# lukifer23/Matrix0

Measured on NVIDIA B200. Metric: MCTS sims/sec, batched self-play, ResNet-24 (BASELINE configs[3]), higher is better.
Workload: dtype fp16

## Files before the change

### matrix0_b200/csrc/nn_fused_kernels.cu

```cuda
#include "nn.cuh"
#include <cuda_fp16.h>

namespace m0 {

__device__ __forceinline__ float fk_act(float x, int act) {
  switch (act) {
    case ACT_RELU: return x > 0.0f ? x : 0.0f;
    case ACT_SILU: return __fdividef(x, 1.0f + __expf(-x));
    default: return x;
  }
}
__device__ __forceinline__ __nv_bfloat16 fk_half(float x, int fp16) {
  if (fp16) {
    __half h = __float2half_rn(x);
    return *reinterpret_cast<__nv_bfloat16*>(&h);
  }
  return __float2bfloat16(x);
}

__device__ __forceinline__ void unpack_half8(const uint4& u, int fp16, float (&f)[8]) {
  const uint32_t w[4] = {u.x, u.y, u.z, u.w};
#pragma unroll
  for (int i = 0; i < 4; ++i) {
    if (fp16) {
      const float2 t = __half22float2(*reinterpret_cast<const __half2*>(&w[i]));
      f[2 * i] = t.x; f[2 * i + 1] = t.y;
    } else {
      const float2 t = __bfloat1622float2(*reinterpret_cast<const __nv_bfloat162*>(&w[i]));
      f[2 * i] = t.x; f[2 * i + 1] = t.y;
    }
  }
}
__device__ __forceinline__ uint32_t fk_pack2(float a, float b, int fp16) {
  if (fp16) {
    __half2 h = __floats2half2_rn(a, b);
    return *reinterpret_cast<uint32_t*>(&h);
  }
  __nv_bfloat162 t = __floats2bfloat162_rn(a, b);
  return *reinterpret_cast<uint32_t*>(&t);
}

__global__ void __launch_bounds__(320, 2)
se_apply_gn_kernel(const __nv_bfloat16* __restrict__ conv_out, const float* __restrict__ gate, float* __restrict__ x,
                   const float* __restrict__ gamma, const float* __restrict__ beta, __nv_bfloat16* __restrict__ a_out, int C, int act, int fp16) {
  __shared__ float s_part[8][40][2];
  const int b = blockIdx.x;
  const int nq = C >> 3;
  const int q = threadIdx.x % nq, rg = threadIdx.x / nq;
  const size_t base = (size_t)b * 64 * C + (size_t)rg * 8 * C + 8 * q;
  float v[8][8];
  if (conv_out) {
    float e[8];
    if (gate) {
      const float4 e0 = *reinterpret_cast<const float4*>(gate + (size_t)b * C + 8 * q);
      const float4 e1 = *reinterpret_cast<const float4*>(gate + (size_t)b * C + 8 * q + 4);
      e[0] = e0.x; e[1] = e0.y; e[2] = e0.z; e[3] = e0.w; e[4] = e1.x; e[5] = e1.y; e[6] = e1.z; e[7] = e1.w;
    } else {
#pragma unroll
      for (int j = 0; j < 8; ++j) e[j] = 1.0f;
    }
    uint4 cv[8];
#pragma unroll
    for (int r = 0; r < 8; ++r) cv[r] = __ldg(reinterpret_cast<const uint4*>(conv_out + base + (size_t)r * C));
#pragma unroll
    for (int r = 0; r < 8; ++r) {
      const float4 x0 = *reinterpret_cast<const float4*>(x + base + (size_t)r * C);
      const float4 x1 = *reinterpret_cast<const float4*>(x + base + (size_t)r * C + 4);
      float c[8];
      unpack_half8(cv[r], fp16, c);
      v[r][0] = fmaf(c[0], e[0], x0.x); v[r][1] = fmaf(c[1], e[1], x0.y); v[r][2] = fmaf(c[2], e[2], x0.z); v[r][3] = fmaf(c[3], e[3], x0.w);
      v[r][4] = fmaf(c[4], e[4], x1.x); v[r][5] = fmaf(c[5], e[5], x1.y); v[r][6] = fmaf(c[6], e[6], x1.z); v[r][7] = fmaf(c[7], e[7], x1.w);
    }
#pragma unroll
    for (int r = 0; r < 8; ++r) {
      *reinterpret_cast<float4*>(x + base + (size_t)r * C) = make_float4(v[r][0], v[r][1], v[r][2], v[r][3]);
      *reinterpret_cast<float4*>(x + base + (size_t)r * C + 4) = make_float4(v[r][4], v[r][5], v[r][6], v[r][7]);
    }
  } else {
#pragma unroll
    for (int r = 0; r < 8; ++r) {
      const float4 x0 = *reinterpret_cast<const float4*>(x + base + (size_t)r * C);
      const float4 x1 = *reinterpret_cast<const float4*>(x + base + (size_t)r * C + 4);
      v[r][0] = x0.x; v[r][1] = x0.y; v[r][2] = x0.z; v[r][3] = x0.w; v[r][4] = x1.x; v[r][5] = x1.y; v[r][6] = x1.z; v[r][7] = x1.w;
    }
  }
  if (!a_out) return;
  __nv_bfloat16* ao = a_out + base;
  if (!gamma) {
#pragma unroll
    for (int r = 0; r < 8; ++r)
      *reinterpret_cast<uint4*>(ao + (size_t)r * C) = make_uint4(fk_pack2(v[r][0], v[r][1], fp16), fk_pack2(v[r][2], v[r][3], fp16),
                                                                 fk_pack2(v[r][4], v[r][5], fp16), fk_pack2(v[r][6], v[r][7], fp16));
    return;
  }
  float s = 0.f;
#pragma unroll
  for (int r = 0; r < 8; ++r) s += ((v[r][0] + v[r][1]) + (v[r][2] + v[r][3])) + ((v[r][4] + v[r][5]) + (v[r][6] + v[r][7]));
  s += __shfl_xor_sync(0xFFFFFFFFu, s, 1);
  s_part[rg][q][0] = s;
  __syncthreads();
  float tot = 0.f;
#pragma unroll
  for (int g = 0; g < 8; ++g) tot += s_part[g][q][0];
  const float mean = tot * (1.0f / 1024.0f);
  float d2 = 0.f;
#pragma unroll
  for (int r = 0; r < 8; ++r)
#pragma unroll
    for (int j = 0; j < 8; ++j) {
      const float a = v[r][j] - mean;
      d2 = fmaf(a, a, d2);
    }
  d2 += __shfl_xor_sync(0xFFFFFFFFu, d2, 1);
  s_part[rg][q][1] = d2;
  __syncthreads();
  float vs = 0.f;
#pragma unroll
  for (int g = 0; g < 8; ++g) vs += s_part[g][q][1];
  const float rstd = rsqrtf(vs * (1.0f / 1024.0f) + 1e-5f);
  float gsc[8], bsh[8];
  {
    const float4 g0 = *reinterpret_cast<const float4*>(gamma + 8 * q), g1 = *reinterpret_cast<const float4*>(gamma + 8 * q + 4);
    const float4 b0 = *reinterpret_cast<const float4*>(beta + 8 * q), b1 = *reinterpret_cast<const float4*>(beta + 8 * q + 4);
    const float gg[8] = {g0.x, g0.y, g0.z, g0.w, g1.x, g1.y, g1.z, g1.w};
    const float bb[8] = {b0.x, b0.y, b0.z, b0.w, b1.x, b1.y, b1.z, b1.w};
#pragma unroll
    for (int j = 0; j < 8; ++j) { gsc[j] = gg[j] * rstd; bsh[j] = bb[j] - mean * gsc[j]; }
  }
#pragma unroll
  for (int r = 0; r < 8; ++r) {
    float y[8];
#pragma unroll
    for (int j = 0; j < 8; ++j) y[j] = fk_act(fmaf(v[r][j], gsc[j], bsh[j]), act);
    *reinterpret_cast<uint4*>(ao + (size_t)r * C) =
        make_uint4(fk_pack2(y[0], y[1], fp16), fk_pack2(y[2], y[3], fp16), fk_pack2(y[4], y[5], fp16), fk_pack2(y[6], y[7], fp16));
  }
}

__global__ void __launch_bounds__(320, 2)
gn_act_res_kernel(const float* __restrict__ x, const float* __restrict__ gamma, const float* __restrict__ beta, const float* __restrict__ residual,
                  long long residual_bstride, float* __restrict__ out, __nv_bfloat16* __restrict__ out_half, int C, int act, int fp16) {
  __shared__ float s_part[8][40][2];
  const int b = blockIdx.x;
  const int nq = C >> 3;
  const int q = threadIdx.x % nq, rg = threadIdx.x / nq;
  const size_t off = (size_t)rg * 8 * C + 8 * q;
  const size_t base = (size_t)b * 64 * C + off;
  float v[8][8];
#pragma unroll
  for (int r = 0; r < 8; ++r) {
    const float4 x0 = *reinterpret_cast<const float4*>(x + base + (size_t)r * C);
    const float4 x1 = *reinterpret_cast<const float4*>(x + base + (size_t)r * C + 4);
    v[r][0] = x0.x; v[r][1] = x0.y; v[r][2] = x0.z; v[r][3] = x0.w; v[r][4] = x1.x; v[r][5] = x1.y; v[r][6] = x1.z; v[r][7] = x1.w;
  }
  float s = 0.f;
#pragma unroll
  for (int r = 0; r < 8; ++r) s += ((v[r][0] + v[r][1]) + (v[r][2] + v[r][3])) + ((v[r][4] + v[r][5]) + (v[r][6] + v[r][7]));
  s += __shfl_xor_sync(0xFFFFFFFFu, s, 1);
  s_part[rg][q][0] = s;
  __syncthreads();
  float tot = 0.f;
#pragma unroll
  for (int g = 0; g < 8; ++g) tot += s_part[g][q][0];
  const float mean = tot * (1.0f / 1024.0f);
  float d2 = 0.f;
#pragma unroll
  for (int r = 0; r < 8; ++r)
#pragma unroll
    for (int j = 0; j < 8; ++j) {
      const float a = v[r][j] - mean;
      d2 = fmaf(a, a, d2);
    }
  d2 += __shfl_xor_sync(0xFFFFFFFFu, d2, 1);
  s_part[rg][q][1] = d2;
  __syncthreads();
  float vs = 0.f;
#pragma unroll
  for (int g = 0; g < 8; ++g) vs += s_part[g][q][1];
  const float rstd = rsqrtf(vs * (1.0f / 1024.0f) + 1e-5f);
  float gsc[8], bsh[8];
  {
    const float4 g0 = *reinterpret_cast<const float4*>(gamma + 8 * q), g1 = *reinterpret_cast<const float4*>(gamma + 8 * q + 4);
    const float4 b0 = *reinterpret_cast<const float4*>(beta + 8 * q), b1 = *reinterpret_cast<const float4*>(beta + 8 * q + 4);
    const float gg[8] = {g0.x, g0.y, g0.z, g0.w, g1.x, g1.y, g1.z, g1.w};
    const float bb[8] = {b0.x, b0.y, b0.z, b0.w, b1.x, b1.y, b1.z, b1.w};
#pragma unroll
    for (int j = 0; j < 8; ++j) { gsc[j] = gg[j] * rstd; bsh[j] = bb[j] - mean * gsc[j]; }
  }
  const float* rb = residual ? residual + (size_t)b * residual_bstride + off : nullptr;
#pragma unroll
  for (int r = 0; r < 8; ++r) {
    float y[8];
#pragma unroll
    for (int j = 0; j < 8; ++j) y[j] = fk_act(fmaf(v[r][j], gsc[j], bsh[j]), act);
    if (rb) {
      const float4 r0 = *reinterpret_cast<const float4*>(rb + (size_t)r * C), r1 = *reinterpret_cast<const float4*>(rb + (size_t)r * C + 4);
      y[0] += r0.x; y[1] += r0.y; y[2] += r0.z; y[3] += r0.w; y[4] += r1.x; y[5] += r1.y; y[6] += r1.z; y[7] += r1.w;
    }
    if (out) {
      *reinterpret_cast<float4*>(out + base + (size_t)r * C) = make_float4(y[0], y[1], y[2], y[3]);
      *reinterpret_cast<float4*>(out + base + (size_t)r * C + 4) = make_float4(y[4], y[5], y[6], y[7]);
    }
    if (out_half)
      *reinterpret_cast<uint4*>(out_half + base + (size_t)r * C) =
          make_uint4(fk_pack2(y[0], y[1], fp16), fk_pack2(y[2], y[3], fp16), fk_pack2(y[4], y[5], fp16), fk_pack2(y[6], y[7], fp16));
  }
}

__global__ void planes_to_nhwc_half_kernel(const float* __restrict__ planes, __nv_bfloat16* __restrict__ out, int B, int P, int fp16) {
  const size_t i = (size_t)blockIdx.x * blockDim.x + threadIdx.x;
  if (i >= (size_t)B * 64 * 64) return;
  const int c = (int)(i & 63);
  const int sq = (int)((i >> 6) & 63);
  const size_t b = i >> 12;
  out[i] = c < P ? fk_half(planes[(b * P + c) * 64 + sq], fp16) : fk_half(0.0f, fp16);
}

__global__ void __launch_bounds__(320)
se_gate_kernel(const float* __restrict__ pool, const float* __restrict__ w1t, const float* __restrict__ b1, const float* __restrict__ w2t,
               const float* __restrict__ b2, float* __restrict__ gate, int B, int C, int hid, int act) {
  extern __shared__ float sm[];
  float* s_pool = sm;
  float* s_hid = sm + 16 * C;
  float* s_red = s_hid + 16 * hid;
  const int b0 = blockIdx.x * 16, t = threadIdx.x;
  const int nb = min(16, B - b0);
  for (int i = t; i < 16 * C; i += blockDim.x) {
    const int j = i / C, c = i - j * C;
    float v = 0.f;
    if (j < nb) {
      const float* pp = pool + (size_t)(b0 + j) * 2 * C;
      v = (pp[c] + pp[C + c]) * (1.0f / 64.0f);
    }
    s_pool[c * 16 + j] = v;
  }
  __syncthreads();
  {
    const int parts = blockDim.x / hid;
    const int part = t / hid, u = t - part * hid;
    if (part < parts) {
      float h[16];
#pragma unroll
      for (int j = 0; j < 16; ++j) h[j] = 0.f;
      const int c0 = part * (C / parts), c1 = (part + 1 == parts) ? C : c0 + C / parts;
#pragma unroll 16
      for (int c = c0; c < c1; ++c) {
        const float w = __ldg(w1t + c * hid + u);
        const float4* sp = reinterpret_cast<const float4*>(s_pool + c * 16);
        const float4 p0 = sp[0], p1 = sp[1], p2 = sp[2], p3 = sp[3];
        h[0] = fmaf(w, p0.x, h[0]); h[1] = fmaf(w, p0.y, h[1]); h[2] = fmaf(w, p0.z, h[2]); h[3] = fmaf(w, p0.w, h[3]);
        h[4] = fmaf(w, p1.x, h[4]); h[5] = fmaf(w, p1.y, h[5]); h[6] = fmaf(w, p1.z, h[6]); h[7] = fmaf(w, p1.w, h[7]);
        h[8] = fmaf(w, p2.x, h[8]); h[9] = fmaf(w, p2.y, h[9]); h[10] = fmaf(w, p2.z, h[10]); h[11] = fmaf(w, p2.w, h[11]);
        h[12] = fmaf(w, p3.x, h[12]); h[13] = fmaf(w, p3.y, h[13]); h[14] = fmaf(w, p3.z, h[14]); h[15] = fmaf(w, p3.w, h[15]);
      }
      float4* dst = reinterpret_cast<float4*>(s_red + (part * hid + u) * 16);
      dst[0] = make_float4(h[0], h[1], h[2], h[3]); dst[1] = make_float4(h[4], h[5], h[6], h[7]);
      dst[2] = make_float4(h[8], h[9], h[10], h[11]); dst[3] = make_float4(h[12], h[13], h[14], h[15]);
    }
    __syncthreads();
    for (int o = t; o < hid * 16; o += blockDim.x) {
      const int u2 = o >> 4;
      float a = b1[u2];
      for (int pp = 0; pp < parts; ++pp) a += s_red[pp * hid * 16 + o];
      s_hid[o] = fk_act(a, act);
    }
    __syncthreads();
  }
  for (int c = t; c < C; c += blockDim.x) {
    float z[16];
    const float bias = b2[c];
#pragma unroll
    for (int j = 0; j < 16; ++j) z[j] = bias;
#pragma unroll 16
    for (int u = 0; u < hid; ++u) {
      const float w = __ldg(w2t + u * C + c);
      const float4* sh = reinterpret_cast<const float4*>(s_hid + u * 16);
      const float4 p0 = sh[0], p1 = sh[1], p2 = sh[2], p3 = sh[3];
      z[0] = fmaf(w, p0.x, z[0]); z[1] = fmaf(w, p0.y, z[1]); z[2] = fmaf(w, p0.z, z[2]); z[3] = fmaf(w, p0.w, z[3]);
      z[4] = fmaf(w, p1.x, z[4]); z[5] = fmaf(w, p1.y, z[5]); z[6] = fmaf(w, p1.z, z[6]); z[7] = fmaf(w, p1.w, z[7]);
      z[8] = fmaf(w, p2.x, z[8]); z[9] = fmaf(w, p2.y, z[9]); z[10] = fmaf(w, p2.z, z[10]); z[11] = fmaf(w, p2.w, z[11]);
      z[12] = fmaf(w, p3.x, z[12]); z[13] = fmaf(w, p3.y, z[13]); z[14] = fmaf(w, p3.z, z[14]); z[15] = fmaf(w, p3.w, z[15]);
    }
#pragma unroll
    for (int j = 0; j < 16; ++j)
      if (j < nb) gate[(size_t)(b0 + j) * C + c] = __fdividef(1.0f, 1.0f + __expf(-z[j]));
  }
}

int nn_se_gate(const float* pool, const float* w1t, const float* b1, const float* w2t, const float* b2, float* gate, int B, int C, int hid, int act,
               cudaStream_t s) {
  if (hid <= 0 || hid > 320) { m0_set_error("se_gate: unsupported hidden width %d", hid); return M0_ERR_ARG; }
  const int parts = 320 / hid;
  se_gate_kernel<<<(B + 15) / 16, 320, (size_t)16 * (C + hid + (size_t)parts * hid) * sizeof(float), s>>>(pool, w1t, b1, w2t, b2, gate, B, C, hid, act);
  return m0_check_launch("se_gate");
}

int nn_se_apply_gn(const __nv_bfloat16* conv_out, const float* gate, float* x, const float* gamma, const float* beta, __nv_bfloat16* a_out, int B,
                   int C, int act, cudaStream_t s) {
  if (C > 320 || C % 32 != 0) { m0_set_error("se_apply_gn: unsupported channel count %d", C); return M0_ERR_ARG; }
  if (C % 16 != 0) { m0_set_error("se_apply_gn: channels must be a multiple of 16"); return M0_ERR_ARG; }
  se_apply_gn_kernel<<<B, C, 0, s>>>(conv_out, gate, x, gamma, beta, a_out, C, act, nn_half_format());
  return m0_check_launch("se_apply_gn");
}
int nn_gn_act_res(const float* x, const float* gamma, const float* beta, const float* residual, long long residual_bstride, float* out,
                  __nv_bfloat16* out_half, int B, int C, int act, cudaStream_t s) {
  if (C > 320 || C % 16 != 0) { m0_set_error("gn_act_res: unsupported channel count %d", C); return M0_ERR_ARG; }
  if (act != ACT_NONE && act != ACT_RELU && act != ACT_SILU) { m0_set_error("gn_act_res: unsupported activation %d", act); return M0_ERR_ARG; }
  gn_act_res_kernel<<<B, C, 0, s>>>(x, gamma, beta, residual, residual_bstride, out, out_half, C, act, nn_half_format());
  return m0_check_launch("gn_act_res");
}
__global__ void se_hidden_kernel(const float* __restrict__ part, int splits, long long split_stride, const float* __restrict__ b1,
                                 __nv_bfloat16* __restrict__ hidden, int B, int hid, int ld, int act, int fp16) {
  const int i = blockIdx.x * blockDim.x + threadIdx.x;
  if (i >= B * hid) return;
  const int b = i / hid, u = i - b * hid;
  float a = b1[u];
  for (int ks = 0; ks < splits; ++ks) a += part[(size_t)ks * split_stride + (size_t)b * ld + u];
  hidden[(size_t)b * ld + u] = fk_half(fk_act(a, act), fp16);
}
int nn_se_hidden(const float* part, int splits, long long split_stride, const float* b1, __nv_bfloat16* hidden, int B, int hid, int ld, int act,
                 cudaStream_t s) {
  se_hidden_kernel<<<(B * hid + 255) / 256, 256, 0, s>>>(part, splits, split_stride, b1, hidden, B, hid, ld, act, nn_half_format());
  return m0_check_launch("se_hidden");
}
static constexpr int SE_TAIL_BOARDS = 8;
__global__ void __launch_bounds__(320, 4)
se_tail_kernel(const float* __restrict__ part, int splits, long long split_stride, int ld, const float* __restrict__ b1,
                               const float* __restrict__ w2t, const float* __restrict__ b2, float* __restrict__ gate, int B, int C, int hid, int act) {
  extern __shared__ __align__(16) float s_hid[];
  const int b0 = blockIdx.x * SE_TAIL_BOARDS;
  const int nb = min(SE_TAIL_BOARDS, B - b0);
  for (int i = threadIdx.x; i < SE_TAIL_BOARDS * hid; i += blockDim.x) {
    const int b = i / hid, u = i - b * hid;
    float a = 0.f;
    if (b < nb) {
      a = b1[u];
      for (int ks = 0; ks < splits; ++ks) a += part[(size_t)ks * split_stride + (size_t)(b0 + b) * ld + u];
      a = fk_act(a, act);
    }
    s_hid[u * SE_TAIL_BOARDS + b] = a;
  }
  __syncthreads();
  for (int c = threadIdx.x; c < C; c += blockDim.x) {
    float acc[SE_TAIL_BOARDS];
#pragma unroll
    for (int b = 0; b < SE_TAIL_BOARDS; ++b) acc[b] = 0.f;
    for (int u0 = 0; u0 < hid; u0 += 16) {
      float w[16];
#pragma unroll
      for (int k = 0; k < 16; ++k) w[k] = (u0 + k < hid) ? __ldg(w2t + (size_t)(u0 + k) * C + c) : 0.f;
#pragma unroll
      for (int k = 0; k < 16; ++k) {
        if (u0 + k >= hid) break;
        const float4 h0 = *reinterpret_cast<const float4*>(s_hid + (u0 + k) * SE_TAIL_BOARDS);
        const float4 h1 = *reinterpret_cast<const float4*>(s_hid + (u0 + k) * SE_TAIL_BOARDS + 4);
        acc[0] = fmaf(w[k], h0.x, acc[0]); acc[1] = fmaf(w[k], h0.y, acc[1]); acc[2] = fmaf(w[k], h0.z, acc[2]); acc[3] = fmaf(w[k], h0.w, acc[3]);
        acc[4] = fmaf(w[k], h1.x, acc[4]); acc[5] = fmaf(w[k], h1.y, acc[5]); acc[6] = fmaf(w[k], h1.z, acc[6]); acc[7] = fmaf(w[k], h1.w, acc[7]);
      }
    }
    const float bias = b2[c];
#pragma unroll
    for (int b = 0; b < SE_TAIL_BOARDS; ++b)
      if (b < nb) gate[(size_t)(b0 + b) * C + c] = __fdividef(1.0f, 1.0f + __expf(-(acc[b] + bias)));
  }
}
int nn_se_tail(const float* part, int splits, long long split_stride, int ld, const float* b1, const float* w2t, const float* b2, float* gate, int B,
               int C, int hid, int act, cudaStream_t s) {
  const int threads = C >= 320 ? 320 : ((C + 31) / 32 * 32);
  se_tail_kernel<<<(B + SE_TAIL_BOARDS - 1) / SE_TAIL_BOARDS, threads, (size_t)SE_TAIL_BOARDS * hid * sizeof(float), s>>>(
      part, splits, split_stride, ld, b1, w2t, b2, gate, B, C, hid, act);
  return m0_check_launch("se_tail");
}
__global__ void value_tail_kernel(const float* __restrict__ gate, const float* __restrict__ h, const float* __restrict__ w3, const float* __restrict__ b3,
                                  float* __restrict__ values, int B, int C) {
  const int b = blockIdx.x * (blockDim.x >> 5) + (threadIdx.x >> 5), lane = threadIdx.x & 31;
  if (b >= B) return;
  float acc = 0.f;
  for (int c = lane; c < C; c += 32) acc = fmaf(w3[c], h[(size_t)b * C + c] * gate[(size_t)b * C + c], acc);
  for (int off = 16; off > 0; off >>= 1) acc += __shfl_xor_sync(0xFFFFFFFFu, acc, off);
  if (lane == 0) values[b] = tanhf(acc + b3[0]);
}
int nn_value_tail(const float* gate, const float* h, const float* w3, const float* b3, float* values, int B, int C, cudaStream_t s) {
  value_tail_kernel<<<(B + 7) / 8, 256, 0, s>>>(gate, h, w3, b3, values, B, C);
  return m0_check_launch("value_tail");
}
int nn_planes_to_nhwc_half(const float* planes, __nv_bfloat16* out, int B, int P, cudaStream_t s) {
  const size_t total = (size_t)B * 64 * 64;
  planes_to_nhwc_half_kernel<<<(unsigned)((total + 255) / 256), 256, 0, s>>>(planes, out, B, P, nn_half_format());
  return m0_check_launch("planes_to_nhwc_half");
}

}
```

### matrix0_b200/csrc/nn_tc_kernels.cu

```cuda
#include "net_host.cuh"
#include "tc_gemm.cuh"
#include "tc_conv_pair.cuh"
#include <new>
#include <stdlib.h>
#include <string.h>
#include <stdio.h>
#include <string>
#include <utility>
#include <vector>

using namespace m0;

namespace m0 {
int nn_se_apply_gn(const __nv_bfloat16* conv_out, const float* gate, float* x, const float* gamma, const float* beta, __nv_bfloat16* a_out, int B,
                   int C, int act, cudaStream_t s);
int nn_planes_to_nhwc_half(const float* planes, __nv_bfloat16* out, int B, int P, cudaStream_t s);
int nn_se_hidden(const float* part, int splits, long long split_stride, const float* b1, __nv_bfloat16* hidden, int B, int hid, int ld, int act,
                 cudaStream_t s);
int nn_gn_act_res(const float* x, const float* gamma, const float* beta, const float* residual, long long residual_bstride, float* out,
                  __nv_bfloat16* out_half, int B, int C, int act, cudaStream_t s);
int nn_attention_tc(const void* qkv_half, const float* rel_bias, void* out_half, int B, int C, int heads, float mix, cudaStream_t s);
int nn_se_tail(const float* part, int splits, long long split_stride, int ld, const float* b1, const float* w2t, const float* b2, float* gate, int B,
               int C, int hid, int act, cudaStream_t s);
int nn_value_tail(const float* gate, const float* h, const float* w3, const float* b3, float* values, int B, int C, cudaStream_t s);
int nn_se_gate(const float* pool, const float* w1t, const float* b1, const float* w2t, const float* b2, float* gate, int B, int C, int hid, int act,
               cudaStream_t s);
}

namespace m0 {
__global__ void transpose_f32_kernel(const float* __restrict__ in, float* __restrict__ out, int rows, int cols) {
  int i = blockIdx.x * blockDim.x + threadIdx.x;
  if (i >= rows * cols) return;
  int r = i / cols, c = i % cols;
  out[c * rows + r] = in[i];
}
__global__ void se_fold_kernel(const float* __restrict__ conv_w, const float* __restrict__ w1, float* __restrict__ out, int C, int hid) {
  const int K = 12 * C;
  const int i = blockIdx.x * blockDim.x + threadIdx.x;
  if (i >= hid * K) return;
  const int u = i / K, k = i - u * K;
  const int ci = k % C, j = (k / C) % 6, hb = k / (6 * C);
  unsigned plus = 0, minus = 0;
  switch (j) {
    case 0: plus = 0x1FF; break;
    case 1: minus = hb ? 0x007 : 0x1C0; break;
    case 2: minus = 0x124; break;
    case 3: minus = 0x049; break;
    case 4: plus = hb ? (1u << 2) : (1u << 8); break;
    default: plus = hb ? (1u << 0) : (1u << 6); break;
  }
  float acc = 0.f;
  for (int c = 0; c < C; ++c) {
    const float* wr = conv_w + (size_t)c * 9 * C + ci;
    float wsum = 0.f;
#pragma unroll
    for (int t = 0; t < 9; ++t) {
      if (plus & (1u << t)) wsum += wr[t * C];
      if (minus & (1u << t)) wsum -= wr[t * C];
    }
    acc = fmaf(w1[u * C + c], wsum, acc);
  }
  out[i] = acc * (1.0f / 64.0f);
}
template <typename T>
__global__ void pad_cols_kernel(const T* __restrict__ in, T* __restrict__ out, int rows, int cols, int cols_pad) {
  const int i = blockIdx.x * blockDim.x + threadIdx.x;
  if (i >= rows * cols_pad) return;
  const int r = i / cols_pad, c = i - r * cols_pad;
  out[i] = c < cols ? in[r * cols + c] : T(0);
}
}

namespace {

typedef CUresult (*EncodeTiledFn)(CUtensorMap*, CUtensorMapDataType, cuuint32_t, void*, const cuuint64_t*, const cuuint64_t*, const cuuint32_t*,
                                  const cuuint32_t*, CUtensorMapInterleave, CUtensorMapSwizzle, CUtensorMapL2promotion, CUtensorMapFloatOOBfill);

EncodeTiledFn get_encode() {
  static EncodeTiledFn fn = nullptr;
  if (!fn) {
    void* p = nullptr;
    cudaDriverEntryPointQueryResult q;
    if (cudaGetDriverEntryPoint("cuTensorMapEncodeTiled", &p, cudaEnableDefault, &q) == cudaSuccess && q == cudaDriverEntryPointSuccess)
      fn = reinterpret_cast<EncodeTiledFn>(p);
  }
  return fn;
}

int make_map_2d(CUtensorMap* m, const void* ptr, uint64_t rows, uint64_t cols, uint32_t box_rows) {
  EncodeTiledFn enc = get_encode();
  if (!enc) { m0_set_error("cuTensorMapEncodeTiled is not available from the driver"); return M0_ERR_CUDA; }
  cuuint64_t dims[2] = {cols, rows};
  cuuint64_t strides[1] = {cols * 2};
  cuuint32_t box[2] = {64, box_rows};
  cuuint32_t estr[2] = {1, 1};
  CUresult r = enc(m, CU_TENSOR_MAP_DATA_TYPE_BFLOAT16, 2, const_cast<void*>(ptr), dims, strides, box, estr, CU_TENSOR_MAP_INTERLEAVE_NONE,
                   CU_TENSOR_MAP_SWIZZLE_128B, CU_TENSOR_MAP_L2_PROMOTION_L2_256B, CU_TENSOR_MAP_FLOAT_OOB_FILL_NONE);
  if (r != CUDA_SUCCESS) { m0_set_error("cuTensorMapEncodeTiled(2d %llu x %llu) failed: %d", (unsigned long long)rows, (unsigned long long)cols, (int)r); return M0_ERR_CUDA; }
  return M0_OK;
}

int make_map_nhwc(CUtensorMap* m, const void* ptr, uint64_t boards, uint64_t C, uint32_t box_x = 8) {
  EncodeTiledFn enc = get_encode();
  if (!enc) { m0_set_error("cuTensorMapEncodeTiled is not available from the driver"); return M0_ERR_CUDA; }
  cuuint64_t dims[4] = {C, 8, 8, boards};
  cuuint64_t strides[3] = {C * 2, C * 2 * 8, C * 2 * 64};
  cuuint32_t box[4] = {64, box_x, 8, 2};
  cuuint32_t estr[4] = {1, 1, 1, 1};
  CUresult r = enc(m, CU_TENSOR_MAP_DATA_TYPE_BFLOAT16, 4, const_cast<void*>(ptr), dims, strides, box, estr, CU_TENSOR_MAP_INTERLEAVE_NONE,
                   CU_TENSOR_MAP_SWIZZLE_128B, CU_TENSOR_MAP_L2_PROMOTION_L2_256B, CU_TENSOR_MAP_FLOAT_OOB_FILL_NONE);
  if (r != CUDA_SUCCESS) { m0_set_error("cuTensorMapEncodeTiled(nhwc boards=%llu C=%llu) failed: %d", (unsigned long long)boards, (unsigned long long)C, (int)r); return M0_ERR_CUDA; }
  return M0_OK;
}

int make_map_out(CUtensorMap* m, const void* ptr, uint64_t rows, uint64_t cols, bool fp32, bool swizzle64 = false) {
  EncodeTiledFn enc = get_encode();
  if (!enc) { m0_set_error("cuTensorMapEncodeTiled is not available from the driver"); return M0_ERR_CUDA; }
  cuuint64_t dims[2] = {cols, rows};
  cuuint64_t strides[1] = {cols * (fp32 ? 4 : 2)};
  cuuint32_t box[2] = {16, 32};
  cuuint32_t estr[2] = {1, 1};
  CUresult r = enc(m, fp32 ? CU_TENSOR_MAP_DATA_TYPE_FLOAT32 : CU_TENSOR_MAP_DATA_TYPE_BFLOAT16, 2, const_cast<void*>(ptr), dims, strides, box, estr,
                   CU_TENSOR_MAP_INTERLEAVE_NONE, swizzle64 ? CU_TENSOR_MAP_SWIZZLE_64B : CU_TENSOR_MAP_SWIZZLE_NONE, CU_TENSOR_MAP_L2_PROMOTION_NONE,
                   CU_TENSOR_MAP_FLOAT_OOB_FILL_NONE);
  if (r != CUDA_SUCCESS) { m0_set_error("cuTensorMapEncodeTiled(out %llu x %llu) failed: %d", (unsigned long long)rows, (unsigned long long)cols, (int)r); return M0_ERR_CUDA; }
  return M0_OK;
}

struct TcWeight {
  __nv_bfloat16* w = nullptr;
  CUtensorMap map;
  CUtensorMap map_pair;
  bool pair = false;
  int n = 0, k = 0, n_part = 0, cluster = 1;
  int n_launch = 0;
};

int pick_cluster(int n_part) {
  static int forced = -1;
  if (forced < 0) {
    const char* e = getenv("M0_TC_CLUSTER");
    forced = e ? atoi(e) : 0;
  }
  int cs = forced > 0 ? forced : 2;
  while (cs > 1 && ((n_part / cs) % 8 != 0 || n_part % cs != 0)) cs >>= 1;
  return cs;
}

struct TcBlock {
  TcWeight conv1, conv2, qkv, proj;
  TcWeight se_fold, se_w2;
};

struct TcState {
  int sm_count = 148;
  int max_smem = 0;
  size_t smem_pair[9] = {0, 0, 0, 0, 0, 0, 0, 0, 0};
  size_t smem_gemm = 0;
  TcWeight pst, inter;
  std::vector<TcBlock> blocks;
  float *pool = nullptr, *se_hid = nullptr, *se_gate = nullptr;
  std::vector<float*> se_w1t, se_w2t;
  bool se_fused = false;
  int hid_pad = 0;
  __nv_bfloat16 *prims = nullptr, *se_hid_h = nullptr;
  float* se_part = nullptr;
  int se_splits = 1;
  size_t se_rows = 0;
  CUtensorMap prims_mat, se_hid_mat;
  __nv_bfloat16* planes_h = nullptr;
  __nv_bfloat16* qkv_h = nullptr;
  bool heads_tc = false;
  TcWeight pol_conv, pol_fc1, pol_fc2, val_conv1, val_conv2, val_fc1, val_fc2, val_gate;
  bool val_tail_tc = false;
  int pol_rank_pad = 0;
  __nv_bfloat16 *ph_h = nullptr, *pf_h = nullptr, *vh_h = nullptr;
  __nv_bfloat16 *vf1_h = nullptr, *vf2_h = nullptr;
  CUtensorMap ph_mat, pf_mat, vh_conv_mat, vh_fc_mat, vf1_mat, vf2_mat;
  CUtensorMap planes_conv;
  TcWeight stem;
  int cap = 0;
  __nv_bfloat16 *a1 = nullptr, *a2 = nullptr;
  CUtensorMap a1_conv, a2_conv, a1_mat, a2_mat;
  CUtensorMap a1_convp, a2_convp, planes_convp;
  CUtensorMap x_io;
  const void* x_ptr = nullptr;
  CUtensorMap qkv_out, t2f_out;
  CUtensorMap a1_out, a2_out, t1_out, t2h_out;
  const void *t1_ptr = nullptr, *t2_ptr = nullptr;
  int out_rows = 0;
  std::vector<void*> allocs;
};

struct TcProfiler {
  struct Rec { const char* name; cudaEvent_t a, b; };
  std::vector<Rec> pending;
  std::vector<std::pair<std::string, std::pair<double, long>>> acc;
  int on = -1;
  bool enabled() {
    if (on < 0) {
      const char* e = getenv("M0_TC_PROFILE");
      on = (e && atoi(e)) ? 1 : 0;
      if (on) atexit(&TcProfiler::dump_static);
    }
    return on >= 1;
  }
  void set(int enable) { enabled(); on = enable ? 2 : 0; }
  void reset() { collect(); acc.clear(); }
  static TcProfiler& get() { static TcProfiler p; return p; }
  void begin(const char* name, cudaStream_t s) {
    Rec r; r.name = name;
    cudaEventCreate(&r.a); cudaEventCreate(&r.b);
    cudaEventRecord(r.a, s);
    pending.push_back(r);
  }
  void end(cudaStream_t s) { cudaEventRecord(pending.back().b, s); }
  void collect() {
    for (Rec& r : pending) {
      cudaEventSynchronize(r.b);
      float ms = 0.f;
      cudaEventElapsedTime(&ms, r.a, r.b);
      bool found = false;
      for (auto& kv : acc) if (kv.first == r.name) { kv.second.first += ms; kv.second.second++; found = true; break; }
      if (!found) acc.push_back({r.name, {ms, 1}});
      cudaEventDestroy(r.a); cudaEventDestroy(r.b);
    }
    pending.clear();
  }
  static void dump_static() {
    TcProfiler& p = get();
    double tot = 0;
    for (auto& kv : p.acc) tot += kv.second.first;
    fprintf(stderr, "[m0 tc profile] total %.3f ms\n", tot);
    for (auto& kv : p.acc)
      fprintf(stderr, "[m0 tc profile] %5.1f%%  n=%5ld  avg=%9.1f us  %s\n", 100.0 * kv.second.first / tot, kv.second.second,
              1e3 * kv.second.first / kv.second.second, kv.first.c_str());
  }
};
#define PROF(name, call)                                   \
  do {                                                     \
    TcProfiler& _p = TcProfiler::get();                    \
    if (_p.enabled()) {                                    \
      _p.begin(name, s);                                   \
      int _r = (call);                                     \
      _p.end(s);                                           \
      if (_r != M0_OK) return _r;                          \
    } else {                                               \
      int _r = (call);                                     \
      if (_r != M0_OK) return _r;                          \
    }                                                      \
  } while (0)

#define TRY(x)            \
  do {                    \
    int _r = (x);         \
    if (_r != M0_OK) return _r; \
  } while (0)

int n_part_for(int n) { return n <= 256 ? n : n / 2; }

int kblocks_for(int cin) { return (cin + 63) / 64; }

int env_int(const char* name, int dflt) {
  const char* e = getenv(name);
  return e ? atoi(e) : dflt;
}
int slice_width_for(int n, int dflt) {
  static int forced = -1;
  if (forced < 0) forced = env_int("M0_TC_SLICE", 0);
  if (forced > 0) return (n % forced == 0) ? forced : dflt;
  if (!env_int("M0_TC_ACC2", 1)) return dflt;
  for (int w = 256; w >= 64; w -= 16)
    if (n % w == 0) return w;
  return dflt;
}
bool pair_ok(int n) {
  static int on = -1;
  if (on < 0) on = env_int("M0_TC_PAIR", 1);
  return on && n % 32 == 0 && n >= 64 && n <= 512;
}

struct ConvFusion {
  float* resid_x = nullptr;
  const float* gate = nullptr;
  __nv_bfloat16* prims = nullptr;
  const CUtensorMap* x_map = nullptr;
};

int launch_conv_pair(TcState* st, const CUtensorMap& a_map, const TcWeight& w, int boards, int cin, float* out_f32, __nv_bfloat16* out_half,
                     int ldc, int act, cudaStream_t s, const float* gn_gamma = nullptr, const float* gn_beta = nullptr, float* pool_part = nullptr,
                     const ConvFusion* fuse = nullptr, int conv = 1, int n_slices = 1, const CUtensorMap* out_map = nullptr) {
  tc::ConvPairParams p;
  memset(&p, 0, sizeof(p));
  p.boards = boards;
  p.N = w.n_launch;
  p.kb_per_tap = kblocks_for(cin);
  p.conv = conv;
  p.n_slices = n_slices;
  if (n_slices > 1 && (gn_gamma || pool_part || fuse)) { m0_set_error("pair kernel: fused epilogues need a single slice"); return M0_ERR_ARG; }
  p.fp16 = nn_half_format();
  p.out_f32 = out_f32;
  p.out_half = out_half;
  p.ldc = ldc;
  p.act = act;
  p.gn_gamma = gn_gamma;
  p.gn_beta = gn_beta;
  p.pool_part = pool_part;
  if (fuse) { p.resid_x = fuse->resid_x; p.gate = fuse->gate; p.prims = fuse->prims; }
  static int cap = -1;
  if (cap < 0) cap = env_int("M0_TC_STAGES", 0);
  const int stage_bytes = conv ? tc::CP_A_SLOT + 3 * (w.n_launch / 4) * 128 : (w.n_launch / 4) * 128;
  const int a_res = conv ? 0 : 2 * kblocks_for(cin) * tc::A_TILE_BYTES;
  const int fz = !fuse ? 0 : fuse->resid_x ? 2 : fuse->prims ? 1 : 0;
  const int epi_bytes = fz == 2 ? tc::CP_EPI_BYTES_FUSE : tc::CP_EPI_BYTES;
  int stages = (st->max_smem - 2048 - epi_bytes - a_res) / stage_bytes;
  if (stages > 8) stages = 8;
  if (cap > 0 && stages > cap) stages = cap;
  if (stages < 2) { m0_set_error("pair convolution: stage does not fit in shared memory (N=%d)", w.n_launch); return M0_ERR_ARG; }
  p.stages = stages;
  const size_t smem = (size_t)stages * stage_bytes + a_res + epi_bytes + 1024 + 512;
  const int nch = (w.n_launch / 32 + tc::CP_CSETS - 1) / tc::CP_CSETS;
  if (nch > 4) { m0_set_error("pair kernel: N = %d is too wide", w.n_launch); return M0_ERR_ARG; }
  auto kernel = fz == 2 ? (nch <= 1 ? tc::conv_pair_kernel<1, 2> : nch <= 3 ? tc::conv_pair_kernel<3, 2> : tc::conv_pair_kernel<4, 2>)
                : fz == 1 ? (nch <= 1 ? tc::conv_pair_kernel<1, 1> : nch <= 3 ? tc::conv_pair_kernel<3, 1> : tc::conv_pair_kernel<4, 1>)
                          : (nch <= 1 ? tc::conv_pair_kernel<1, 0> : nch <= 3 ? tc::conv_pair_kernel<3, 0> : tc::conv_pair_kernel<4, 0>);
  const int kidx = (nch <= 1 ? 0 : nch <= 3 ? 1 : 2) + 3 * fz;
  if (smem > st->smem_pair[kidx]) {
    M0_CUDA_TRY(cudaFuncSetAttribute(kernel, cudaFuncAttributeMaxDynamicSharedMemorySize, (int)smem));
    st->smem_pair[kidx] = smem;
  }
  const int tiles = (boards + 3) / 4;
  int clusters = st->sm_count / 2;
  if (clusters > tiles) clusters = tiles;
  cudaLaunchConfig_t cfg;
  memset(&cfg, 0, sizeof(cfg));
  cfg.gridDim = dim3((unsigned)(clusters * 2));
  cfg.blockDim = dim3(tc::CP_THREADS);
  cfg.dynamicSmemBytes = smem;
  cfg.stream = s;
  cudaLaunchAttribute attr[1];
  attr[0].id = cudaLaunchAttributeClusterDimension;
  attr[0].val.clusterDim.x = 2;
  attr[0].val.clusterDim.y = 1;
  attr[0].val.clusterDim.z = 1;
  cfg.attrs = attr;
  cfg.numAttrs = 1;
  if (fuse && fuse->resid_x && (!fuse->x_map || (out_half && !out_map))) { m0_set_error("pair kernel: the residual epilogue needs the x and output tensor maps"); return M0_ERR_ARG; }
  p.out_tma = (out_map && !(fuse && fuse->prims)) ? 1 : 0;
  M0_CUDA_TRY(cudaLaunchKernelEx(&cfg, kernel, a_map, w.map_pair, out_map ? *out_map : a_map, (fuse && fuse->x_map) ? *fuse->x_map : a_map, p));
  return m0_check_launch("conv_pair_kernel");
}

int make_weight(TcState* st, TcWeight* out, const float* w_f32, int n, int k, int n_launch, cudaStream_t s, int taps = 1) {
  const int cin = k / taps, cin_pad = taps > 1 ? kblocks_for(cin) * 64 : cin;
  k = taps * cin_pad;
  out->n = n;
  out->k = k;
  out->n_part = n_part_for(n_launch);
  out->cluster = pick_cluster(out->n_part);
  void* p = nullptr;
  M0_CUDA_TRY(cudaMalloc(&p, (size_t)n * k * 2));
  st->allocs.push_back(p);
  out->w = (__nv_bfloat16*)p;
  if (cin_pad != cin) {
    float* padded = nullptr;
    M0_CUDA_TRY(cudaMallocAsync((void**)&padded, (size_t)n * k * 4, s));
    pad_cols_kernel<float><<<(n * k + 255) / 256, 256, 0, s>>>(w_f32, padded, n * taps, cin, cin_pad);
    int rc = m0_check_launch("pad_taps");
    if (rc == M0_OK) rc = nn_f32_to_bf16(padded, out->w, (size_t)n * k, s);
    cudaFreeAsync(padded, s);
    TRY(rc);
  } else {
    TRY(nn_f32_to_bf16(w_f32, out->w, (size_t)n * k, s));
  }
  out->n_launch = n_launch;
  out->pair = pair_ok(n_launch) && n % n_launch == 0;
  if (out->pair) TRY(make_map_2d(&out->map_pair, out->w, (uint64_t)n, (uint64_t)k, (uint32_t)(n_launch / 4)));
  return make_map_2d(&out->map, out->w, (uint64_t)n, (uint64_t)k, (uint32_t)(out->n_part / out->cluster));
}

int pow2_cols(int n) {
  int c = 32;
  while (c < n) c <<= 1;
  return c;
}

int launch_gemm(TcState* st, const CUtensorMap& a_map, const TcWeight& w, int M, int conv, int taps, int cin, int w_row0, int N, float* out_f32,
                __nv_bfloat16* out_bf16, int ldc, int col0, const float* bias, int act, float scale, cudaStream_t s,
                const float* gn_gamma = nullptr, const float* gn_beta = nullptr, float* pool_part = nullptr, int n_store = -1, int n_slices = 1,
                int k_splits = 1, long long split_stride = 0) {
  tc::GemmParams p;
  memset(&p, 0, sizeof(p));
  p.M = M;
  p.N = N;
  p.n_slices = n_slices;
  p.k_splits = k_splits;
  p.split_stride = split_stride;
  if (k_splits > 1 && (out_bf16 || bias || act != ACT_NONE || gn_gamma || pool_part || (taps * kblocks_for(cin)) % k_splits != 0 || !out_f32)) {
    m0_set_error("tensor-core GEMM: split-K needs a plain fp32 output and a K range divisible into whole k-blocks");
    return M0_ERR_ARG;
  }
  p.n_store = n_store >= 0 ? n_store : N * n_slices;
  if (w.n_part > N || N % w.n_part != 0) { m0_set_error("tensor-core GEMM: launch width %d does not match the weight map box %d", N, w.n_part); return M0_ERR_ARG; }
  p.n_part = w.n_part;
  p.taps = taps;
  p.kb_per_tap = kblocks_for(cin);
  p.conv = conv;
  p.w_row0 = w_row0;
  {
    static int acc2 = -1;
    if (acc2 < 0) acc2 = env_int("M0_TC_ACC2", 1);
    const int stride = (N + 31) / 32 * 32;
    p.acc_stages = (acc2 && 2 * stride <= 512 && !gn_gamma) ? 2 : 1;
    p.acc_stride = stride;
    p.tmem_cols = pow2_cols(p.acc_stages * stride);
  }
  p.out_f32 = out_f32;
  p.out_bf16 = out_bf16;
  p.ldc = ldc;
  p.col0 = col0;
  p.bias = bias;
  p.act = act;
  p.scale = scale;
  p.gn_gamma = gn_gamma;
  p.gn_beta = gn_beta;
  p.pool_part = pool_part;
  if ((gn_gamma || pool_part) && (w_row0 != 0 || N % 32 != 0)) { m0_set_error("fused epilogue needs the full channel range"); return M0_ERR_ARG; }
  p.cluster = w.cluster;
  p.fp16 = nn_half_format();
  const int stage_bytes = tc::A_TILE_BYTES + N * tc::BK * 2;
  int stages = (st->max_smem - 2048 - tc::EPI_STAGE_BYTES) / stage_bytes;
  if (stages > 6) stages = 6;
  {
    static int cap = -1;
    if (cap < 0) { const char* e = getenv("M0_TC_STAGES"); cap = e ? atoi(e) : 0; }
    if (cap > 0 && stages > cap) stages = cap;
  }
  if (stages < 2) { m0_set_error("tensor-core GEMM: tile does not fit in shared memory (N=%d)", N); return M0_ERR_ARG; }
  p.stages = stages;
  const size_t smem = (size_t)stages * stage_bytes + tc::EPI_STAGE_BYTES + 1024 + 256;
  if (smem > st->smem_gemm) {
    M0_CUDA_TRY(cudaFuncSetAttribute(tc::gemm_tc_kernel, cudaFuncAttributeMaxDynamicSharedMemorySize, (int)smem));
    st->smem_gemm = smem;
  }
  const int tiles = (M + tc::BM - 1) / tc::BM;
  const int cs = w.cluster;
  const int groups = (tiles + cs - 1) / cs;
  int clusters = st->sm_count / cs;
  if (clusters > groups * n_slices * k_splits) clusters = groups * n_slices * k_splits;
  cudaLaunchConfig_t cfg;
  memset(&cfg, 0, sizeof(cfg));
  cfg.gridDim = dim3((unsigned)(clusters * cs));
  cfg.blockDim = dim3(tc::NUM_THREADS);
  cfg.dynamicSmemBytes = smem;
  cfg.stream = s;
  cudaLaunchAttribute attr[1];
  attr[0].id = cudaLaunchAttributeClusterDimension;
  attr[0].val.clusterDim.x = (unsigned)cs;
  attr[0].val.clusterDim.y = 1;
  attr[0].val.clusterDim.z = 1;
  cfg.attrs = attr;
  cfg.numAttrs = 1;
  M0_CUDA_TRY(cudaLaunchKernelEx(&cfg, tc::gemm_tc_kernel, a_map, w.map, p));
  return m0_check_launch("gemm_tc_kernel");
}

int conv3x3(TcState* st, const CUtensorMap& a_map, const CUtensorMap& a_map_pair, const TcWeight& w, int B, int cin, float* out_f32,
            __nv_bfloat16* out_half, int act, cudaStream_t s, const float* gn_gamma = nullptr, const float* gn_beta = nullptr,
            float* pool_part = nullptr, const ConvFusion* fuse = nullptr, const CUtensorMap* out_map = nullptr) {
  if (w.pair) return launch_conv_pair(st, a_map_pair, w, B, cin, out_f32, out_half, w.n, act, s, gn_gamma, gn_beta, pool_part, fuse, 1, 1, out_map);
  if (fuse) { m0_set_error("fused SE / residual epilogue needs the CTA-pair convolution"); return M0_ERR_ARG; }
  return launch_gemm(st, a_map, w, B * 64, 1, 9, cin, 0, w.n, out_f32, out_half, w.n, 0, nullptr, act, 1.0f, s, gn_gamma, gn_beta, pool_part);
}

int gemm_rows64(TcState* st, const CUtensorMap& a_mat, const TcWeight& w, int B, int cin, float* out_f32, __nv_bfloat16* out_half, int ldc,
                cudaStream_t s, const CUtensorMap* out_map = nullptr) {
  const int n_slices = w.n / w.n_launch;
  static int pg = -1;
  if (pg < 0) pg = env_int("M0_TC_PAIR_GEMM", 0);
  if (pg && w.pair && cin <= 320)
    return launch_conv_pair(st, a_mat, w, B, cin, out_f32, out_half, ldc, ACT_NONE, s, nullptr, nullptr, nullptr, nullptr, 0, n_slices, out_map);
  return launch_gemm(st, a_mat, w, B * 64, 0, 1, cin, 0, w.n_launch, out_f32, out_half, ldc, 0, nullptr, ACT_NONE, 1.0f, s, nullptr, nullptr, nullptr, -1,
                     n_slices);
}

int tc_reserve(m0_net* n, TcState* st, int B) {
  const int need = (B + 1) & ~1;
  if (need <= st->cap) return M0_OK;
  const size_t C = n->cfg.channels;
  if (st->a1) cudaFree(st->a1);
  if (st->a2) cudaFree(st->a2);
  if (st->pool) cudaFree(st->pool);
  if (st->se_hid) cudaFree(st->se_hid);
  if (st->se_gate) cudaFree(st->se_gate);
  if (st->planes_h) cudaFree(st->planes_h);
  if (st->qkv_h) cudaFree(st->qkv_h);
  if (st->ph_h) cudaFree(st->ph_h);
  if (st->pf_h) cudaFree(st->pf_h);
  if (st->vh_h) cudaFree(st->vh_h);
  if (st->vf1_h) cudaFree(st->vf1_h);
  if (st->vf2_h) cudaFree(st->vf2_h);
  st->vf1_h = st->vf2_h = nullptr;
  if (st->prims) cudaFree(st->prims);
  if (st->se_hid_h) cudaFree(st->se_hid_h);
  if (st->se_part) cudaFree(st->se_part);
  st->se_part = nullptr;
  st->prims = st->se_hid_h = nullptr;
  st->qkv_h = st->ph_h = st->pf_h = st->vh_h = nullptr;
  st->a1 = st->a2 = nullptr;
  st->pool = st->se_hid = st->se_gate = nullptr;
  st->planes_h = nullptr;
  st->cap = 0;
  M0_CUDA_TRY(cudaMalloc((void**)&st->pool, (size_t)need * 2 * C * 4));
  M0_CUDA_TRY(cudaMalloc((void**)&st->se_hid, (size_t)need * (n->cfg.se_hidden > 0 ? n->cfg.se_hidden : 1) * 4));
  M0_CUDA_TRY(cudaMalloc((void**)&st->se_gate, (size_t)need * C * 4));
  M0_CUDA_TRY(cudaMalloc((void**)&st->planes_h, (size_t)need * 64 * 64 * 2));
  M0_CUDA_TRY(cudaMalloc((void**)&st->qkv_h, (size_t)need * 64 * 3 * C * 2));
  if (st->heads_tc) {
    const size_t rp = (size_t)st->pol_rank_pad;
    M0_CUDA_TRY(cudaMalloc((void**)&st->ph_h, (size_t)need * 4096 * 2));
    M0_CUDA_TRY(cudaMalloc((void**)&st->pf_h, (size_t)need * rp * 2));
    M0_CUDA_TRY(cudaMalloc((void**)&st->vh_h, (size_t)need * 8192 * 2));
    M0_CUDA_TRY(cudaMemset(st->pf_h, 0, (size_t)need * rp * 2));
    TRY(make_map_2d(&st->ph_mat, st->ph_h, (uint64_t)need, 4096, 128));
    TRY(make_map_2d(&st->pf_mat, st->pf_h, (uint64_t)need, rp, 128));
    TRY(make_map_2d(&st->vh_conv_mat, st->vh_h, (uint64_t)need * 64, 128, 128));
    TRY(make_map_2d(&st->vh_fc_mat, st->vh_h, (uint64_t)need, 8192, 128));
    if (st->val_tail_tc) {
      M0_CUDA_TRY(cudaMalloc((void**)&st->vf1_h, (size_t)need * 2 * C * 2));
      M0_CUDA_TRY(cudaMalloc((void**)&st->vf2_h, (size_t)need * C * 2));
      TRY(make_map_2d(&st->vf1_mat, st->vf1_h, (uint64_t)need, 2 * C, 128));
      TRY(make_map_2d(&st->vf2_mat, st->vf2_h, (uint64_t)need, C, 128));
    }
  }
  if (st->se_fused && n->cfg.se) {
    const size_t rows = ((size_t)need + 127) / 128 * 128;
    M0_CUDA_TRY(cudaMalloc((void**)&st->prims, rows * 12 * C * 2));
    M0_CUDA_TRY(cudaMalloc((void**)&st->se_hid_h, rows * st->hid_pad * 2));
    M0_CUDA_TRY(cudaMemset(st->prims, 0, rows * 12 * C * 2));
    M0_CUDA_TRY(cudaMemset(st->se_hid_h, 0, rows * st->hid_pad * 2));
    const int kblocks = 12 * (int)C / 64;
    st->se_splits = kblocks % 4 == 0 ? 4 : kblocks % 3 == 0 ? 3 : kblocks % 2 == 0 ? 2 : 1;
    st->se_rows = rows;
    M0_CUDA_TRY(cudaMalloc((void**)&st->se_part, (size_t)st->se_splits * rows * st->hid_pad * 4));
    TRY(make_map_2d(&st->prims_mat, st->prims, rows, 12 * C, 128));
    TRY(make_map_2d(&st->se_hid_mat, st->se_hid_h, rows, (uint64_t)st->hid_pad, 128));
  }
  M0_CUDA_TRY(cudaMemset(st->planes_h, 0, (size_t)need * 64 * 64 * 2));
  TRY(make_map_nhwc(&st->planes_conv, st->planes_h, need, 64));
  TRY(make_map_nhwc(&st->planes_convp, st->planes_h, need, 64, 10));
  M0_CUDA_TRY(cudaMalloc((void**)&st->a1, (size_t)need * 64 * C * 2));
  M0_CUDA_TRY(cudaMalloc((void**)&st->a2, (size_t)need * 64 * C * 2));
  M0_CUDA_TRY(cudaMemset(st->a1, 0, (size_t)need * 64 * C * 2));
  M0_CUDA_TRY(cudaMemset(st->a2, 0, (size_t)need * 64 * C * 2));
  TRY(make_map_nhwc(&st->a1_conv, st->a1, need, C));
  TRY(make_map_nhwc(&st->a2_conv, st->a2, need, C));
  TRY(make_map_nhwc(&st->a1_convp, st->a1, need, C, 10));
  TRY(make_map_nhwc(&st->a2_convp, st->a2, need, C, 10));
  st->t1_ptr = st->t2_ptr = nullptr;
  TRY(make_map_2d(&st->a1_mat, st->a1, (uint64_t)need * 64, C, 128));
  TRY(make_map_2d(&st->a2_mat, st->a2, (uint64_t)need * 64, C, 128));
  st->cap = need;
  return M0_OK;
}

}

namespace m0 {

struct TcStates {
  TcState* st[2] = {nullptr, nullptr};
};

int tc_net_prepare(::m0_net* n, cudaStream_t s) {
  if (!n->tc) n->tc = new (std::nothrow) TcStates();
  TcStates* all = (TcStates*)n->tc;
  if (!all) { m0_set_error("out of host memory"); return M0_ERR_ARG; }
  const int fmt = nn_half_format();
  if (all->st[fmt]) return M0_OK;
  const m0_net_config& c = n->cfg;
  if (c.channels % 32 != 0 || c.channels < 64 || c.channels > 320) {
    m0_set_error("16-bit tensor-core path needs channels %% 32 == 0 and 64 <= channels <= 320 (got %d)", c.channels);
    return M0_ERR_ARG;
  }
  TcState* st = new (std::nothrow) TcState();
  if (!st) { m0_set_error("out of host memory"); return M0_ERR_ARG; }
  cudaDeviceGetAttribute(&st->sm_count, cudaDevAttrMultiProcessorCount, n->device);
  cudaDeviceGetAttribute(&st->max_smem, cudaDevAttrMaxSharedMemoryPerBlockOptin, n->device);
  const int C = c.channels;
  int rc = M0_OK;
  do {
    if ((rc = make_weight(st, &st->stem, n->w.stem_w, C, 9 * c.planes, C, s, 9)) != M0_OK) break;
    if (c.se) {
      st->se_w1t.resize(c.blocks, nullptr);
      st->se_w2t.resize(c.blocks, nullptr);
      const int hc = c.se_hidden * C;
      for (int i = 0; i < c.blocks && rc == M0_OK; ++i) {
        float *w1t = nullptr, *w2t = nullptr;
        if ((rc = m0_check_cuda(cudaMalloc((void**)&w1t, (size_t)hc * 4), "cudaMalloc se")) != M0_OK) break;
        st->allocs.push_back(w1t);
        if ((rc = m0_check_cuda(cudaMalloc((void**)&w2t, (size_t)hc * 4), "cudaMalloc se")) != M0_OK) break;
        st->allocs.push_back(w2t);
        st->se_w1t[i] = w1t;
        st->se_w2t[i] = w2t;
        transpose_f32_kernel<<<(hc + 255) / 256, 256, 0, s>>>(n->w.blocks[i].se_w1, w1t, c.se_hidden, C);
        transpose_f32_kernel<<<(hc + 255) / 256, 256, 0, s>>>(n->w.blocks[i].se_w2, w2t, C, c.se_hidden);
        rc = m0_check_launch("transpose_se");
      }
      if (rc != M0_OK) break;
    }
    if (c.policy_factor_rank > 0 && c.policy_factor_rank % 16 == 0 && c.policy_factor_rank <= 320) {
      const int r = c.policy_factor_rank, rp = (r + 63) / 64 * 64;
      st->pol_rank_pad = rp;
      float* w2p = nullptr;
      const int ps_pad = (c.policy_size + 319) / 320 * 320;
      if ((rc = m0_check_cuda(cudaMalloc((void**)&w2p, (size_t)ps_pad * rp * 4), "cudaMalloc pol_fc2")) != M0_OK) break;
      st->allocs.push_back(w2p);
      if ((rc = m0_check_cuda(cudaMemsetAsync(w2p, 0, (size_t)ps_pad * rp * 4, s), "memset")) != M0_OK) break;
      if ((rc = m0_check_cuda(cudaMemcpy2DAsync(w2p, (size_t)rp * 4, n->w.pol_fc2_w, (size_t)r * 4, (size_t)r * 4, c.policy_size,
                                                cudaMemcpyDeviceToDevice, s), "pad pol_fc2")) != M0_OK) break;
      if ((rc = make_weight(st, &st->pol_conv, n->w.pol_conv_w, 64, C, 64, s)) != M0_OK) break;
      if ((rc = make_weight(st, &st->pol_fc1, n->w.pol_fc1_w, r, 4096, r, s)) != M0_OK) break;
      if ((rc = make_weight(st, &st->pol_fc2, w2p, ps_pad, rp, 320, s)) != M0_OK) break;
      if ((rc = make_weight(st, &st->val_conv1, n->w.val_conv1_w, 128, C, 128, s)) != M0_OK) break;
      if ((rc = make_weight(st, &st->val_conv2, n->w.val_conv2_w, 128, 128, 128, s)) != M0_OK) break;
      const int fc1_launch = n_part_for(C) % 32 == 0 ? C : slice_width_for(C, C);
      if ((rc = make_weight(st, &st->val_fc1, n->w.val_fc1_w, 2 * C, 8192, fc1_launch, s)) != M0_OK) break;
      if (env_int("M0_TC_VALUE_TAIL", 1)) {
        if ((rc = make_weight(st, &st->val_fc2, n->w.val_fc2_w, C, 2 * C, slice_width_for(C, C), s)) != M0_OK) break;
        if ((rc = make_weight(st, &st->val_gate, n->w.val_gate_w, C, C, slice_width_for(C, C), s)) != M0_OK) break;
        st->val_tail_tc = true;
      }
      st->heads_tc = true;
    }
    if (c.chess_features) {
      if (c.piece_square_tables && (rc = make_weight(st, &st->pst, n->w.pst_w, C, C, env_int("M0_TC_SLICE_PROJ", 1) ? slice_width_for(C, C) : C, s)) != M0_OK) break;
      if ((rc = make_weight(st, &st->inter, n->w.inter_w, C, 9 * C, C, s, 9)) != M0_OK) break;
    }
    st->hid_pad = (c.se_hidden + 63) / 64 * 64;
    st->se_fused = env_int("M0_TC_FUSE_SE", 1) != 0 && pair_ok(C) && (!c.se || c.se_hidden <= 256);
    st->blocks.resize(c.blocks);
    for (int i = 0; i < c.blocks && rc == M0_OK; ++i) {
      const m0_block_weights& b = n->w.blocks[i];
      if ((rc = make_weight(st, &st->blocks[i].conv1, b.conv1_w, C, 9 * C, C, s, 9)) != M0_OK) break;
      if ((rc = make_weight(st, &st->blocks[i].conv2, b.conv2_w, C, 9 * C, C, s, 9)) != M0_OK) break;
      if (st->se_fused && c.se) {
        const int hid = c.se_hidden, hid16 = (hid + 15) / 16 * 16, K = 12 * C, hp = st->hid_pad;
        float *fold = nullptr, *w2p = nullptr;
        if ((rc = m0_check_cuda(cudaMalloc((void**)&fold, (size_t)hid16 * K * 4), "cudaMalloc se_fold")) != M0_OK) break;
        st->allocs.push_back(fold);
        if ((rc = m0_check_cuda(cudaMemsetAsync(fold, 0, (size_t)hid16 * K * 4, s), "memset se_fold")) != M0_OK) break;
        if ((rc = m0_check_cuda(cudaMalloc((void**)&w2p, (size_t)C * hp * 4), "cudaMalloc se_w2")) != M0_OK) break;
        st->allocs.push_back(w2p);
        se_fold_kernel<<<(hid * K + 255) / 256, 256, 0, s>>>(b.conv2_w, b.se_w1, fold, C, hid);
        pad_cols_kernel<float><<<(C * hp + 255) / 256, 256, 0, s>>>(b.se_w2, w2p, C, hid, hp);
        if ((rc = m0_check_launch("se_fold")) != M0_OK) break;
        if ((rc = make_weight(st, &st->blocks[i].se_fold, fold, hid16, K, hid16, s)) != M0_OK) break;
        if ((rc = make_weight(st, &st->blocks[i].se_w2, w2p, C, hp, C, s)) != M0_OK) break;
      }
      if (b.has_attention) {
        if ((rc = make_weight(st, &st->blocks[i].qkv, b.att_qkv_w, 3 * C, C, slice_width_for(3 * C, C), s)) != M0_OK) break;
        if ((rc = make_weight(st, &st->blocks[i].proj, b.att_proj_w, C, C, env_int("M0_TC_SLICE_PROJ", 1) ? slice_width_for(C, C) : C, s)) != M0_OK) break;
      }
    }
  } while (0);
  if (rc != M0_OK) {
    for (void* p : st->allocs) cudaFree(p);
    delete st;
    return rc;
  }
  all->st[fmt] = st;
  return M0_OK;
}

void tc_net_release(::m0_net* n) {
  TcStates* all = (TcStates*)n->tc;
  if (!all) return;
  for (int f = 0; f < 2; ++f) {
    TcState* st = all->st[f];
    if (!st) continue;
    for (void* p : st->allocs) cudaFree(p);
    if (st->a1) cudaFree(st->a1);
    if (st->a2) cudaFree(st->a2);
    if (st->pool) cudaFree(st->pool);
    if (st->se_hid) cudaFree(st->se_hid);
    if (st->se_gate) cudaFree(st->se_gate);
    if (st->planes_h) cudaFree(st->planes_h);
    if (st->qkv_h) cudaFree(st->qkv_h);
    if (st->ph_h) cudaFree(st->ph_h);
    if (st->pf_h) cudaFree(st->pf_h);
    if (st->vh_h) cudaFree(st->vh_h);
    if (st->vf1_h) cudaFree(st->vf1_h);
    if (st->vf2_h) cudaFree(st->vf2_h);
    if (st->prims) cudaFree(st->prims);
    if (st->se_hid_h) cudaFree(st->se_hid_h);
    if (st->se_part) cudaFree(st->se_part);
    delete st;
  }
  delete all;
  n->tc = nullptr;
}

int tc_net_forward(::m0_net* n, const float* planes, int B, float* logits, float* values, cudaStream_t s) {
  TcState* st = ((TcStates*)n->tc)->st[nn_half_format()];
  TRY(net_ws_reserve(n, B));
  TRY(tc_reserve(n, st, B));
  const m0_net_config& c = n->cfg;
  const m0_net_weights& w = n->w;
  const int C = c.channels, M = B * 64, act = c.activation;
  const float* none = nullptr;
  if (st->t1_ptr != n->t1 || st->t2_ptr != n->t2 || st->x_ptr != n->x || st->out_rows != M) {
    TRY(make_map_out(&st->a1_out, st->a1, (uint64_t)M, C, false));
    TRY(make_map_out(&st->a2_out, st->a2, (uint64_t)M, C, false));
    TRY(make_map_out(&st->t1_out, n->t1, (uint64_t)M, C, true));
    TRY(make_map_out(&st->t2h_out, n->t2, (uint64_t)M, C, false));
    TRY(make_map_out(&st->t2f_out, n->t2, (uint64_t)M, C, true));
    TRY(make_map_out(&st->qkv_out, st->qkv_h, (uint64_t)M, 3 * (uint64_t)C, false));
    TRY(make_map_out(&st->x_io, n->x, (uint64_t)M, C, true, true));
    st->x_ptr = n->x;
    st->t1_ptr = n->t1;
    st->t2_ptr = n->t2;
    st->out_rows = M;
  }
  PROF("planes_to_nhwc_half", nn_planes_to_nhwc_half(planes, st->planes_h, B, c.planes, s));
  PROF("conv_other", conv3x3(st, st->planes_conv, st->planes_convp, st->stem, B, 64, n->t1, nullptr, ACT_NONE, s, nullptr, nullptr, nullptr, nullptr, &st->t1_out));
  if (c.chess_features) {
    PROF("gn_act_res", nn_gn_act_res(n->t1, w.stem_gn_w, w.stem_gn_b, w.pos_enc, 0, n->x, st->a1, B, C, act, s));
    float* cur = n->x;
    if (c.piece_square_tables) {
      PROF("gemm_pst", gemm_rows64(st, st->a1_mat, st->pst, B, C, n->t1, nullptr, C, s, &st->t1_out));
      PROF("gn_act_res", nn_gn_act_res(n->t1, w.pst_gn_w, w.pst_gn_b, n->x, (long long)64 * C, n->t2, st->a1, B, C, act, s));
      cur = n->t2;
    }
    PROF("conv_other", conv3x3(st, st->a1_conv, st->a1_convp, st->inter, B, C, n->t1, nullptr, ACT_NONE, s, nullptr, nullptr, nullptr, nullptr, &st->t1_out));
    PROF("gn_act_res", nn_gn_act_res(n->t1, w.inter_gn_w, w.inter_gn_b, cur, (long long)64 * C, n->x, nullptr, B, C, act, s));
  } else {
    PROF("groupnorm_f32", nn_groupnorm_f32(n->t1, w.stem_gn_w, w.stem_gn_b, nullptr, 0, n->x, B, C, act, s));
  }
  if (c.blocks > 0) PROF("se_apply_gn", nn_se_apply_gn(nullptr, nullptr, n->x, w.blocks[0].gn1_w, w.blocks[0].gn1_b, st->a1, B, C, act, s));
  int att_seen = 0;
  bool heads_input_ready = false;
  const int stride = c.infer_attention_stride > 1 ? c.infer_attention_stride : 1;
  for (int i = 0; i < c.blocks; ++i) {
    const m0_block_weights& b = w.blocks[i];
    const TcBlock& tb = st->blocks[i];
    bool run_att = false;
    if (b.has_attention) {
      att_seen++;
      run_att = (att_seen % stride) == 0;
    }
    const bool last = (i + 1 == c.blocks);
    const bool fuse_next = !last && !run_att;
    const bool tc_att = run_att && C == c.attention_heads * 16;
    __nv_bfloat16* next_a = (fuse_next || run_att) ? st->a1 : nullptr;
    if (st->se_fused) {
      ConvFusion f1;
      f1.prims = c.se ? st->prims : nullptr;
      PROF("conv1+gn", conv3x3(st, st->a1_conv, st->a1_convp, tb.conv1, B, C, nullptr, st->a2, act, s, b.gn2_w, b.gn2_b, nullptr, &f1));
      if (c.se) {
        static int se_nosplit = -1;
        if (se_nosplit < 0) se_nosplit = env_int("M0_SE_NOSPLIT", 0);
        if (se_nosplit) {
          PROF("se_fc1", launch_gemm(st, st->prims_mat, tb.se_fold, B, 0, 1, 12 * C, 0, tb.se_fold.n, nullptr, st->se_hid_h, st->hid_pad, 0, b.se_b1, act, 1.0f, s,
                                     nullptr, nullptr, nullptr, c.se_hidden));
        } else {
          PROF("se_fc1", launch_gemm(st, st->prims_mat, tb.se_fold, B, 0, 1, 12 * C, 0, tb.se_fold.n, st->se_part, nullptr, st->hid_pad, 0, none, ACT_NONE, 1.0f, s,
                                     nullptr, nullptr, nullptr, c.se_hidden, 1, st->se_splits, (long long)st->se_rows * st->hid_pad));
          static int se_tail = -1;
          if (se_tail < 0) se_tail = env_int("M0_SE_TAIL", 1);
          if (se_tail) {
            PROF("se_tail", nn_se_tail(st->se_part, st->se_splits, (long long)st->se_rows * st->hid_pad, st->hid_pad, b.se_b1, st->se_w2t[i], b.se_b2,
                                       st->se_gate, B, C, c.se_hidden, act, s));
            goto se_done;
          }
          PROF("se_hidden", nn_se_hidden(st->se_part, st->se_splits, (long long)st->se_rows * st->hid_pad, b.se_b1, st->se_hid_h, B, c.se_hidden, st->hid_pad, act, s));
        }
        PROF("se_fc2", launch_gemm(st, st->se_hid_mat, tb.se_w2, B, 0, 1, st->hid_pad, 0, C, st->se_gate, nullptr, C, 0, b.se_b2, ACT_SIGMOID, 1.0f, s));
      se_done:;
      }
      ConvFusion f2;
      f2.resid_x = n->x;
      f2.gate = c.se ? st->se_gate : nullptr;
      f2.x_map = &st->x_io;
      PROF("conv2+se+res+gn", conv3x3(st, st->a2_conv, st->a2_convp, tb.conv2, B, C, nullptr, next_a, act, s, fuse_next ? w.blocks[i + 1].gn1_w : nullptr,
                                      fuse_next ? w.blocks[i + 1].gn1_b : nullptr, nullptr, &f2, next_a ? &st->a1_out : nullptr));
    } else {
      PROF("conv1+gn", conv3x3(st, st->a1_conv, st->a1_convp, tb.conv1, B, C, nullptr, st->a2, act, s, b.gn2_w, b.gn2_b, nullptr, nullptr, &st->a2_out));
      __nv_bfloat16* t2h = reinterpret_cast<__nv_bfloat16*>(n->t2);
      PROF("conv2+pool", conv3x3(st, st->a2_conv, st->a2_convp, tb.conv2, B, C, nullptr, t2h, ACT_NONE, s, nullptr, nullptr, c.se ? st->pool : nullptr, nullptr,
                                 &st->t2h_out));
      const float* gate = nullptr;
      if (c.se) {
        PROF("se_gate", nn_se_gate(st->pool, st->se_w1t[i], b.se_b1, st->se_w2t[i], b.se_b2, st->se_gate, B, C, c.se_hidden, act, s));
        gate = st->se_gate;
      }
      PROF("se_apply_gn", nn_se_apply_gn(t2h, gate, n->x, fuse_next ? w.blocks[i + 1].gn1_w : nullptr, fuse_next ? w.blocks[i + 1].gn1_b : nullptr,
                                         next_a, B, C, act, s));
    }
    if (run_att) {
      const float* rb = c.attention_relbias ? b.att_rel_bias : nullptr;
      if (tc_att) {
        PROF("gemm_qkv", gemm_rows64(st, st->a1_mat, tb.qkv, B, C, nullptr, st->qkv_h, 3 * C, s, &st->qkv_out));
        PROF("attention_tc", nn_attention_tc(st->qkv_h, rb, st->a2, B, C, c.attention_heads, c.attention_unmasked_mix, s));
      } else {
        PROF("gemm_qkv", gemm_rows64(st, st->a1_mat, tb.qkv, B, C, n->qkv, nullptr, 3 * C, s));
        PROF("attention_f32", nn_attention_f32(n->qkv, rb, n->t1, B, C, c.attention_heads, c.attention_unmasked_mix, s));
        PROF("f32_to_bf16", nn_f32_to_bf16(n->t1, st->a2, (size_t)M * C, s));
      }
      static int proj_f32 = -1;
      if (proj_f32 < 0) proj_f32 = env_int("M0_TC_PROJ_F32", 0);
      const bool fused_ln = C % 32 == 0 && C <= 320;
      const bool proj_half = fused_ln && !proj_f32;
      if (proj_half) PROF("gemm_proj", gemm_rows64(st, st->a2_mat, tb.proj, B, C, nullptr, reinterpret_cast<__nv_bfloat16*>(n->t2), C, s, &st->t2h_out));
      else PROF("gemm_proj", gemm_rows64(st, st->a2_mat, tb.proj, B, C, n->t2, nullptr, C, s, &st->t2f_out));
      if (fused_ln) {
        heads_input_ready = last && st->heads_tc;
        PROF("ln_res_gn", nn_ln_res_gn(n->t2, proj_half ? 1 : 0, n->x, b.att_ln_w, b.att_ln_b, last ? nullptr : w.blocks[i + 1].gn1_w,
                                       last ? nullptr : w.blocks[i + 1].gn1_b, (last && !st->heads_tc) ? nullptr : st->a1, B, C, act, s));
      } else {
        PROF("layernorm_residual_f32", nn_layernorm_residual_f32(n->t2, n->x, b.att_ln_w, b.att_ln_b, n->x, M, C, s));
        if (!last) PROF("se_apply_gn", nn_se_apply_gn(nullptr, nullptr, n->x, w.blocks[i + 1].gn1_w, w.blocks[i + 1].gn1_b, st->a1, B, C, act, s));
      }
    }
  }
  if (!st->heads_tc) return net_forward_heads_f32(n, B, logits, values, s);
  const int vact = c.value_activation, r = c.policy_factor_rank, rp = st->pol_rank_pad;
  if (!heads_input_ready) PROF("f32_to_bf16", nn_f32_to_bf16(n->x, st->a1, (size_t)M * C, s));
  PROF("gemm_pol_conv", launch_gemm(st, st->a1_mat, st->pol_conv, M, 0, 1, C, 0, 64, n->t1, nullptr, 64, 0, none, ACT_NONE, 1.0f, s));
  PROF("gn_act_res", nn_gn_act_res(n->t1, w.pol_gn_w, w.pol_gn_b, nullptr, 0, nullptr, st->ph_h, B, 64, act, s));
  PROF("gemm_pol_fc1", launch_gemm(st, st->ph_mat, st->pol_fc1, B, 0, 1, 4096, 0, r, nullptr, st->pf_h, rp, 0, w.pol_fc1_b, ACT_RELU, 1.0f, s));
  PROF("gemm_pol_fc2", launch_gemm(st, st->pf_mat, st->pol_fc2, B, 0, 1, rp, 0, 320, logits, nullptr, c.policy_size, 0, w.pol_fc2_b, ACT_NONE,
                                   w.policy_logit_scale, s, nullptr, nullptr, nullptr, c.policy_size, (c.policy_size + 319) / 320));
  PROF("gemm_val_conv1", launch_gemm(st, st->a1_mat, st->val_conv1, M, 0, 1, C, 0, 128, n->vh1, nullptr, 128, 0, none, ACT_NONE, 1.0f, s));
  PROF("gn_act_res", nn_gn_act_res(n->vh1, w.val_gn1_w, w.val_gn1_b, nullptr, 0, nullptr, st->vh_h, B, 128, act, s));
  PROF("gemm_val_conv2", launch_gemm(st, st->vh_conv_mat, st->val_conv2, M, 0, 1, 128, 0, 128, n->vh1, nullptr, 128, 0, none, ACT_NONE, 1.0f, s));
  PROF("gn_act_res", nn_gn_act_res(n->vh1, w.val_gn2_w, w.val_gn2_b, nullptr, 0, nullptr, st->vh_h, B, 128, act, s));
  if (st->val_tail_tc) {
    PROF("gemm_val_fc1", launch_gemm(st, st->vh_fc_mat, st->val_fc1, B, 0, 1, 8192, 0, st->val_fc1.n_launch, nullptr, st->vf1_h, 2 * C, 0, w.val_fc1_b, vact,
                                     1.0f, s, nullptr, nullptr, nullptr, -1, 2 * C / st->val_fc1.n_launch));
    PROF("gemm_val_fc2", launch_gemm(st, st->vf1_mat, st->val_fc2, B, 0, 1, 2 * C, 0, st->val_fc2.n_launch, n->vf2, st->vf2_h, C, 0, w.val_fc2_b, vact, 1.0f, s,
                                     nullptr, nullptr, nullptr, -1, C / st->val_fc2.n_launch));
    PROF("gemm_val_gate", launch_gemm(st, st->vf2_mat, st->val_gate, B, 0, 1, C, 0, st->val_gate.n_launch, n->vg, nullptr, C, 0, w.val_gate_b, ACT_SIGMOID, 1.0f,
                                      s, nullptr, nullptr, nullptr, -1, C / st->val_gate.n_launch));
    PROF("value_tail", nn_value_tail(n->vg, n->vf2, w.val_fc3_w, w.val_fc3_b, values, B, C, s));
  } else {
    PROF("gemm_val_fc1", launch_gemm(st, st->vh_fc_mat, st->val_fc1, B, 0, 1, 8192, 0, st->val_fc1.n_launch, n->vf1, nullptr, 2 * C, 0, w.val_fc1_b, vact, 1.0f,
                                     s, nullptr, nullptr, nullptr, -1, 2 * C / st->val_fc1.n_launch));
    PROF("gemm_f32", nn_gemm_f32(A_DIRECT, n->vf1, w.val_fc2_w, w.val_fc2_b, nullptr, n->vf2, B, C, 2 * C, 2 * C, C, 0, vact, 1.0f, s));
    PROF("gemm_f32", nn_gemm_f32(A_DIRECT, n->vf2, w.val_gate_w, w.val_gate_b, n->vf2, n->vg, B, C, C, C, C, 0, ACT_SIGMOID, 1.0f, s));
    PROF("gemm_f32", nn_gemm_f32(A_DIRECT, n->vg, w.val_fc3_w, w.val_fc3_b, nullptr, values, B, 1, C, C, 1, 0, ACT_TANH, 1.0f, s));
  }
  if (TcProfiler::get().enabled()) TcProfiler::get().collect();
  return M0_OK;
}

}

extern "C" int m0_tc_conv(const uint16_t* d_act_bf16, const uint16_t* d_w_bf16, int boards, int cin, int n, int taps, float* d_out_f32,
                          void* stream) {
  if (!d_act_bf16 || !d_w_bf16 || !d_out_f32 || boards <= 0 || (boards & 1) || cin <= 0 || cin % 32 != 0 || n % 16 != 0 || n > 320 ||
      (taps != 1 && taps != 9)) {
    m0_set_error("m0_tc_conv: invalid argument (boards even, cin %% 32 == 0, n %% 16 == 0, n <= 320, taps in {1, 9})");
    return M0_ERR_ARG;
  }
  struct FormatGuard {
    int saved;
    FormatGuard() : saved(nn_half_format()) { nn_set_half_format(0); }
    ~FormatGuard() { nn_set_half_format(saved); }
  } format_guard;
  static TcState st;
  static int st_dev = -1;
  int dev = 0;
  cudaGetDevice(&dev);
  if (dev != st_dev) {
    for (size_t& v : st.smem_pair) v = 0;
    st.smem_gemm = 0;
    st_dev = dev;
  }
  cudaDeviceGetAttribute(&st.sm_count, cudaDevAttrMultiProcessorCount, dev);
  cudaDeviceGetAttribute(&st.max_smem, cudaDevAttrMaxSharedMemoryPerBlockOptin, dev);
  const cudaStream_t s = (cudaStream_t)stream;
  const int kw = taps * kblocks_for(cin) * 64;
  void* w_pad = nullptr;
  if (taps == 9 && kw != taps * cin) {
    M0_CUDA_TRY(cudaMallocAsync(&w_pad, (size_t)n * kw * 2, s));
    pad_cols_kernel<uint16_t><<<(n * kw + 255) / 256, 256, 0, s>>>(d_w_bf16, (uint16_t*)w_pad, n * taps, cin, kw / taps);
    const int rc = m0_check_launch("pad_taps");
    if (rc != M0_OK) { cudaFreeAsync(w_pad, s); return rc; }
  }
  auto run = [&](const void* wp, int k) -> int {
    TcWeight w;
    w.w = (__nv_bfloat16*)wp;
    w.n = n;
    w.k = k;
    w.n_part = n_part_for(n);
    w.cluster = pick_cluster(w.n_part);
    TRY(make_map_2d(&w.map, wp, (uint64_t)n, (uint64_t)k, (uint32_t)(w.n_part / w.cluster)));
    CUtensorMap a;
    w.n_launch = n;
    if (taps == 9 && pair_ok(n)) {
      w.pair = true;
      TRY(make_map_2d(&w.map_pair, wp, (uint64_t)n, (uint64_t)k, (uint32_t)(n / 4)));
      TRY(make_map_nhwc(&a, d_act_bf16, (uint64_t)boards, (uint64_t)cin, 10));
      CUtensorMap om;
      TRY(make_map_out(&om, d_out_f32, (uint64_t)boards * 64, (uint64_t)n, true));
      return launch_conv_pair(&st, a, w, boards, cin, d_out_f32, nullptr, n, ACT_NONE, s, nullptr, nullptr, nullptr, nullptr, 1, 1, &om);
    }
    if (taps == 1 && pair_ok(n) && cin <= 320) {
      w.pair = true;
      TRY(make_map_2d(&w.map_pair, wp, (uint64_t)n, (uint64_t)cin, (uint32_t)(n / 4)));
      TRY(make_map_2d(&a, d_act_bf16, (uint64_t)boards * 64, (uint64_t)cin, 128));
      return launch_conv_pair(&st, a, w, boards, cin, d_out_f32, nullptr, n, ACT_NONE, s, nullptr, nullptr, nullptr, nullptr, 0, 1);
    }
    if (taps == 9) TRY(make_map_nhwc(&a, d_act_bf16, (uint64_t)boards, (uint64_t)cin));
    else TRY(make_map_2d(&a, d_act_bf16, (uint64_t)boards * 64, (uint64_t)cin, 128));
    return launch_gemm(&st, a, w, boards * 64, taps == 9 ? 1 : 0, taps, cin, 0, n, d_out_f32, nullptr, n, 0, nullptr, ACT_NONE, 1.0f, s);
  };
  const int rc = w_pad ? run(w_pad, kw) : run(d_w_bf16, taps * cin);
  if (w_pad) cudaFreeAsync(w_pad, s);
  return rc;
}

extern "C" int m0_profile_enable(int enable) {
  TcProfiler& p = TcProfiler::get();
  p.reset();
  p.set(enable);
  return M0_OK;
}
extern "C" int m0_profile_get(const char* name, double* total_ms, long long* launches) {
  TcProfiler& p = TcProfiler::get();
  p.collect();
  double ms = 0;
  long long cnt = 0;
  for (auto& kv : p.acc)
    if (!name || kv.first == name) { ms += kv.second.first; cnt += kv.second.second; }
  if (total_ms) *total_ms = ms;
  if (launches) *launches = cnt;
  return M0_OK;
}
```

### matrix0_b200/csrc/tc_conv_pair.cuh

```cuda
#pragma once
#include "tc_gemm.cuh"

namespace m0 {
namespace tc {

struct ConvPairParams {
  int boards;
  int N;
  int kb_per_tap;
  int conv;
  int n_slices;
  int stages;
  int fp16;
  float* out_f32;
  __nv_bfloat16* out_half;
  int ldc;
  int out_tma;
  int act;
  const float* gn_gamma;
  const float* gn_beta;
  float* pool_part;
  float* resid_x;
  const float* gate;
  __nv_bfloat16* prims;
};

static constexpr int CP_EPI_WARP0 = 4;
static constexpr int CP_EPI_WARPS = 16;
static constexpr int CP_CSETS = CP_EPI_WARPS / 4;
static constexpr int CP_THREADS = (CP_EPI_WARP0 + CP_EPI_WARPS) * 32;
static constexpr int CP_REGS_CTRL = 40, CP_REGS_EPI = 104;
static constexpr int CP_A_SLOT = 160 * 128;
static constexpr int CP_EPI_BYTES = CP_EPI_WARPS * 2048 + 2 * 512 * 4 + 2 * 4 * 16 * 2 * 4 + CP_EPI_WARPS * 64 * 4;
static constexpr int CP_EPI_BYTES_FUSE = CP_EPI_BYTES + CP_EPI_WARPS * 2048;

__device__ __forceinline__ uint32_t mapa_u32(uint32_t addr, uint32_t rank) {
  uint32_t r;
  asm volatile("mapa.shared::cluster.u32 %0, %1, %2;" : "=r"(r) : "r"(addr), "r"(rank));
  return r;
}
__device__ __forceinline__ void mbar_arrive_cluster(uint32_t cluster_addr) {
  asm volatile("mbarrier.arrive.release.cluster.shared::cluster.b64 _, [%0];" ::"r"(cluster_addr) : "memory");
}
__device__ __forceinline__ void tma_load_4d_pair(void* dst, const CUtensorMap* map, uint32_t bar, int c0, int c1, int c2, int c3) {
  asm volatile("cp.async.bulk.tensor.4d.cta_group::2.shared::cluster.global.mbarrier::complete_tx::bytes [%0], [%1, {%3, %4, %5, %6}], [%2];" ::"r"(
                   smem_u32(dst)),
               "l"(reinterpret_cast<uint64_t>(map)), "r"(bar), "r"(c0), "r"(c1), "r"(c2), "r"(c3)
               : "memory");
}
__device__ __forceinline__ void tma_load_2d_pair(void* dst, const CUtensorMap* map, uint32_t bar, int c0, int c1) {
  asm volatile("cp.async.bulk.tensor.2d.cta_group::2.shared::cluster.global.mbarrier::complete_tx::bytes [%0], [%1, {%3, %4}], [%2];" ::"r"(
                   smem_u32(dst)),
               "l"(reinterpret_cast<uint64_t>(map)), "r"(bar), "r"(c0), "r"(c1)
               : "memory");
}
__device__ __forceinline__ void tmem_alloc_pair(uint32_t* dst_smem, uint32_t cols) {
  asm volatile("tcgen05.alloc.cta_group::2.sync.aligned.shared::cta.b32 [%0], %1;" ::"r"(smem_u32(dst_smem)), "r"(cols) : "memory");
}
__device__ __forceinline__ void tmem_relinquish_pair() { asm volatile("tcgen05.relinquish_alloc_permit.cta_group::2.sync.aligned;" ::: "memory"); }
__device__ __forceinline__ void tmem_dealloc_pair(uint32_t addr, uint32_t cols) {
  asm volatile("tcgen05.dealloc.cta_group::2.sync.aligned.b32 %0, %1;" ::"r"(addr), "r"(cols) : "memory");
}
__device__ __forceinline__ void umma_pair(uint32_t tmem_d, uint64_t desc_a, uint64_t desc_b, uint32_t idesc, uint32_t accumulate) {
  asm volatile(
      "{\n\t"
      ".reg .pred p;\n\t"
      "setp.ne.b32 p, %4, 0;\n\t"
      "tcgen05.mma.cta_group::2.kind::f16 [%0], %1, %2, %3, p;\n\t"
      "}\n" ::"r"(tmem_d),
      "l"(desc_a), "l"(desc_b), "r"(idesc), "r"(accumulate)
      : "memory");
}
__device__ __forceinline__ void umma_commit_pair(uint64_t* bar, uint16_t cta_mask) {
  asm volatile("tcgen05.commit.cta_group::2.mbarrier::arrive::one.shared::cluster.multicast::cluster.b64 [%0], %1;" ::"r"(smem_u32(bar)),
               "h"(cta_mask)
               : "memory");
}
__device__ __forceinline__ void tmem_ld_32x16(uint32_t taddr, uint32_t (&r)[16]) {
  asm volatile(
      "tcgen05.ld.sync.aligned.32x32b.x16.b32 "
      "{%0, %1, %2, %3, %4, %5, %6, %7, %8, %9, %10, %11, %12, %13, %14, %15}, [%16];"
      : "=r"(r[0]), "=r"(r[1]), "=r"(r[2]), "=r"(r[3]), "=r"(r[4]), "=r"(r[5]), "=r"(r[6]), "=r"(r[7]), "=r"(r[8]), "=r"(r[9]), "=r"(r[10]),
        "=r"(r[11]), "=r"(r[12]), "=r"(r[13]), "=r"(r[14]), "=r"(r[15])
      : "r"(taddr));
}
__device__ __forceinline__ void tma_store_2d(const CUtensorMap* map, const void* smem_src, int c0, int c1) {
  asm volatile("cp.async.bulk.tensor.2d.global.shared::cta.bulk_group [%0, {%2, %3}], [%1];" ::"l"(reinterpret_cast<uint64_t>(map)),
               "r"(smem_u32(smem_src)), "r"(c0), "r"(c1)
               : "memory");
}
__device__ __forceinline__ void tma_store_commit() { asm volatile("cp.async.bulk.commit_group;" ::: "memory"); }
template <int N>
__device__ __forceinline__ void tma_store_wait_read() { asm volatile("cp.async.bulk.wait_group.read %0;" ::"n"(N) : "memory"); }
__device__ __forceinline__ uint64_t make_smem_desc_sbo(uint32_t smem_addr, uint32_t sbo_bytes) {
  return (uint64_t)((smem_addr >> 4) & 0x3FFFu) | (1ull << 16) | ((uint64_t)(sbo_bytes >> 4) << 32) | (1ull << 46) | (2ull << 61);
}

template <int NCH, int FUSE>
__global__ void __launch_bounds__(CP_THREADS, 1)
conv_pair_kernel(const __grid_constant__ CUtensorMap tma_a, const __grid_constant__ CUtensorMap tma_w, const __grid_constant__ CUtensorMap tma_out,
                 const __grid_constant__ CUtensorMap tma_x, const ConvPairParams p) {
  extern __shared__ __align__(1024) uint8_t smem_raw[];
  uint8_t* smem = reinterpret_cast<uint8_t*>((reinterpret_cast<uintptr_t>(smem_raw) + 1023) & ~uintptr_t(1023));
  const int nh = p.N >> 1, nq = p.N >> 2;
  const int wq_bytes = nq * 128;
  const int a_res_bytes = p.conv ? 0 : p.kb_per_tap * A_TILE_BYTES;
  const int stage_bytes = p.conv ? CP_A_SLOT + 3 * wq_bytes : wq_bytes;
  uint8_t* a_res = smem;
  smem += 2 * (size_t)a_res_bytes;
  const int ns2 = 2 * (p.n_slices > 1 ? p.n_slices : 1);
  float* epi_stage = reinterpret_cast<float*>(smem + (size_t)p.stages * stage_bytes);
  float* s_gamma = epi_stage + CP_EPI_WARPS * (FUSE == 2 ? 1024 : 512);
  float* s_beta = s_gamma + 512;
  float* s_stats = s_beta + 512;
  float* s_gate = s_stats + 256;
  uint64_t* full_bar = reinterpret_cast<uint64_t*>(s_gate + CP_EPI_WARPS * 64);
  uint64_t* empty_bar = full_bar + p.stages;
  uint64_t* tmem_full_bar = empty_bar + p.stages;
  uint64_t* tmem_empty_bar = tmem_full_bar + 2;
  uint64_t* a_full_bar = tmem_empty_bar + 2;
  uint64_t* a_empty_bar = a_full_bar + 2;
  uint64_t* x_bar = a_empty_bar + 2;
  uint32_t* tmem_slot = reinterpret_cast<uint32_t*>(x_bar + 2 * CP_EPI_WARPS);

  const int warp = threadIdx.x >> 5, lane = threadIdx.x & 31;
  const int rank = (int)cluster_ctarank();
  const int num_tiles = (p.boards + 3) >> 2;
  const int num_clusters = gridDim.x >> 1;
  const int cluster_id = blockIdx.x >> 1;
  const int steps = p.conv ? p.kb_per_tap * 3 : p.kb_per_tap;

  if (warp == 0 && lane == 0) {
    tma_prefetch_desc(&tma_a);
    tma_prefetch_desc(&tma_w);
    for (int s = 0; s < p.stages; ++s) {
      mbar_init(&full_bar[s], 1);
      mbar_init(&empty_bar[s], 1);
    }
    for (int b = 0; b < 2; ++b) {
      mbar_init(&tmem_full_bar[b], 1);
      mbar_init(&tmem_empty_bar[b], 2 * CP_EPI_WARPS);
      mbar_init(&a_full_bar[b], 1);
      mbar_init(&a_empty_bar[b], 1);
    }
    for (int i = 0; i < 2 * CP_EPI_WARPS; ++i) mbar_init(&x_bar[i], 1);
    fence_barrier_init();
  }
  if (warp == 1) {
    tmem_alloc_pair(tmem_slot, 512);
    tmem_relinquish_pair();
  }
  tc_fence_before();
  __syncthreads();
  cluster_sync_all();
  tc_fence_after();
  const uint32_t tmem_base = *tmem_slot;

  if (warp < CP_EPI_WARP0) {
   asm volatile("setmaxnreg.dec.sync.aligned.u32 %0;" ::"n"(CP_REGS_CTRL));
   if (warp == 0) {
    if (lane == 0) {
      const uint32_t lead_full = mapa_u32(smem_u32(full_bar), 0);
      int stage = 0;
      uint32_t phase = 0;
      const uint32_t lead_afull = mapa_u32(smem_u32(a_full_bar), 0);
      auto load_a_tile = [&](int t, int it) {
        const int ab = it & 1;
        mbar_wait(&a_empty_bar[ab], (uint32_t)((it >> 1) & 1) ^ 1u);
        if (rank == 0) mbar_expect_tx(&a_full_bar[ab], (uint32_t)(2 * a_res_bytes));
        for (int kb = 0; kb < p.kb_per_tap; ++kb)
          tma_load_2d_pair(a_res + (size_t)ab * a_res_bytes + (size_t)kb * A_TILE_BYTES, &tma_a, lead_afull + (uint32_t)ab * 8u, kb * BK,
                           (t * 4 + rank * 2) * 64);
      };
      int it = 0;
      if (!p.conv && cluster_id < num_tiles) load_a_tile(cluster_id, 0);
      for (int t = cluster_id; t < num_tiles; t += num_clusters, ++it) {
        const int board0 = t * 4 + rank * 2;
        if (!p.conv && t + num_clusters < num_tiles) load_a_tile(t + num_clusters, it + 1);
        for (int u2 = 0; u2 < ns2; ++u2) {
          const int w_row = (u2 >> 1) * p.N + (u2 & 1) * nh + rank * nq;
          if (p.conv) {
            for (int kc = 0; kc < p.kb_per_tap; ++kc) {
              for (int dyi = 0; dyi < 3; ++dyi) {
                mbar_wait(&empty_bar[stage], phase ^ 1);
                if (rank == 0) mbar_expect_tx(&full_bar[stage], (uint32_t)(2 * stage_bytes));
                const uint32_t bar = lead_full + (uint32_t)stage * 8u;
                uint8_t* a_dst = smem + (size_t)stage * stage_bytes;
                tma_load_4d_pair(a_dst, &tma_a, bar, kc * BK, -1, dyi - 1, board0);
#pragma unroll
                for (int dxi = 0; dxi < 3; ++dxi)
                  tma_load_2d_pair(a_dst + CP_A_SLOT + dxi * wq_bytes, &tma_w, bar, ((dyi * 3 + dxi) * p.kb_per_tap + kc) * BK, w_row);
                if (++stage == p.stages) { stage = 0; phase ^= 1; }
              }
            }
          } else {
            for (int kb = 0; kb < p.kb_per_tap; ++kb) {
              mbar_wait(&empty_bar[stage], phase ^ 1);
              if (rank == 0) mbar_expect_tx(&full_bar[stage], (uint32_t)(2 * stage_bytes));
              tma_load_2d_pair(smem + (size_t)stage * stage_bytes, &tma_w, lead_full + (uint32_t)stage * 8u, kb * BK, w_row);
              if (++stage == p.stages) { stage = 0; phase ^= 1; }
            }
          }
        }
      }
    }
  } else if (warp == 1) {
    if (rank == 0) {
      const uint32_t idesc = make_idesc_bf16(256, nh, p.fp16);
      const uint32_t smem_base = smem_u32(smem);
      int stage = 0;
      uint32_t phase = 0, unit = 0;
      int it = 0;
      for (int t = cluster_id; t < num_tiles; t += num_clusters, ++it) {
        const uint32_t a_tile = smem_u32(a_res) + (uint32_t)(it & 1) * (uint32_t)a_res_bytes;
        if (!p.conv) {
          mbar_wait(&a_full_bar[it & 1], (uint32_t)(it >> 1) & 1u);
          tc_fence_after();
        }
        for (int u2 = 0; u2 < ns2; ++u2, ++unit) {
          const uint32_t buf = unit & 1u;
          mbar_wait(&tmem_empty_bar[buf], ((unit >> 1) & 1u) ^ 1u);
          tc_fence_after();
          const uint32_t d = tmem_base + buf * 256u;
          for (int step = 0; step < steps; ++step) {
            mbar_wait(&full_bar[stage], phase);
            tc_fence_after();
            const uint32_t a_addr = smem_base + (uint32_t)stage * (uint32_t)stage_bytes;
            if (elect_one()) {
              if (p.conv) {
#pragma unroll
                for (int dxi = 0; dxi < 3; ++dxi) {
                  const uint64_t adesc = make_smem_desc_sbo(a_addr + dxi * 128, 1280);
                  const uint64_t bdesc = make_smem_desc_sbo(a_addr + CP_A_SLOT + dxi * wq_bytes, 1024);
#pragma unroll
                  for (int k = 0; k < BK / 16; ++k) umma_pair(d, adesc + 2 * k, bdesc + 2 * k, idesc, (step > 0 || dxi > 0 || k > 0) ? 1u : 0u);
                }
              } else {
                const uint64_t adesc = make_smem_desc_sbo(a_tile + (uint32_t)step * A_TILE_BYTES, 1024);
                const uint64_t bdesc = make_smem_desc_sbo(a_addr, 1024);
#pragma unroll
                for (int k = 0; k < BK / 16; ++k) umma_pair(d, adesc + 2 * k, bdesc + 2 * k, idesc, (step > 0 || k > 0) ? 1u : 0u);
              }
              umma_commit_pair(&empty_bar[stage], 3);
            }
            __syncwarp();
            if (++stage == p.stages) { stage = 0; phase ^= 1; }
          }
          if (elect_one()) {
            umma_commit_pair(&tmem_full_bar[buf], 3);
            if (!p.conv && u2 == ns2 - 1) umma_commit_pair(&a_empty_bar[it & 1], 3);
          }
          __syncwarp();
        }
      }
    }
   }
  } else {
    asm volatile("setmaxnreg.inc.sync.aligned.u32 %0;" ::"n"(CP_REGS_EPI));
    const int quarter = warp & 3;
    const int cset = (warp - CP_EPI_WARP0) >> 2;
    uint8_t* wtile = reinterpret_cast<uint8_t*>(epi_stage) + (size_t)(warp - CP_EPI_WARP0) * (FUSE == 2 ? 4096 : 2048);
    float* stg = reinterpret_cast<float*>(wtile);
    uint8_t* xin = wtile;
    uint8_t* xout = wtile;
    uint64_t* xbar = x_bar + (warp - CP_EPI_WARP0) * 2;
    uint32_t xuse[2] = {0, 0};
    float* wgate = s_gate + (warp - CP_EPI_WARP0) * (NCH * 16);
    const bool fused_gn = p.gn_gamma != nullptr;
    const bool resid = FUSE == 2 && p.resid_x != nullptr;
    const bool want_prims = FUSE == 1 && p.prims != nullptr;
    const int epi_tid = ((warp - CP_EPI_WARP0) << 5) | lane;
    const uint32_t lead_empty = mapa_u32(smem_u32(tmem_empty_bar), 0);
    const int nchunks = nh >> 4;
    const int M = p.boards * 64;
    const int act = p.act;
    if (fused_gn) {
      for (int c = epi_tid; c < p.N; c += CP_EPI_WARPS * 32) { s_gamma[c] = p.gn_gamma[c]; s_beta[c] = p.gn_beta[c]; }
      asm volatile("bar.sync 1, %0;" ::"n"(CP_EPI_WARPS * 32) : "memory");
    }
    uint32_t unit = 0, nstore = 0;
    for (int t = cluster_id; t < num_tiles; t += num_clusters) {
      for (int u2 = 0; u2 < ns2; ++u2, ++unit) {
        const int h = u2 & 1, cbase = (u2 >> 1) * p.N + h * nh;
        const uint32_t buf = unit & 1u;
        const int row0 = t * 256 + rank * 128 + quarter * 32;
        const int m_lane = row0 + lane;
        if (resid) {
          if (lane == 0) {
            tma_store_wait_read<0>();
#pragma unroll
            for (int k = 0; k < 2; ++k)
              if (k < NCH && cset + CP_CSETS * k < nchunks) {
                mbar_expect_tx(&xbar[k], 2048);
                tma_load_2d(xin + k * 2048, &tma_x, &xbar[k], cbase + (cset + CP_CSETS * k) * 16, row0);
              }
          }
          if (p.gate) {
            const int bq = row0 >> 6;
            const int k = lane >> 2, q = lane & 3, ci = cset + CP_CSETS * k;
            if (k < NCH && ci < nchunks && row0 < M)
              *reinterpret_cast<float4*>(wgate + k * 16 + 4 * q) = __ldg(reinterpret_cast<const float4*>(p.gate + (size_t)bq * p.N + h * nh + ci * 16 + 4 * q));
          }
        }
        mbar_wait(&tmem_full_bar[buf], (unit >> 1) & 1u);
        tc_fence_after();
        const uint32_t tmem_row = tmem_base + buf * 256u + ((uint32_t)(quarter * 32) << 16);
        float* stats = s_stats + buf * 128;
        uint32_t r[NCH][16];
#pragma unroll
        for (int k = 0; k < NCH; ++k)
          if (cset + CP_CSETS * k < nchunks) tmem_ld_32x16(tmem_row + (uint32_t)((cset + CP_CSETS * k) * 16), r[k]);
        tmem_ld_wait();
        tc_fence_before();
        __syncwarp();
        if (lane == 0) mbar_arrive_cluster(lead_empty + buf * 8u);
        if (resid) {
          const int sw = (lane >> 1) & 3;
#pragma unroll
          for (int k = 0; k < NCH; ++k) {
            const int ci = cset + CP_CSETS * k;
            if (ci >= nchunks) break;
            const int col = cbase + ci * 16;
            const int xb = k & 1;
            mbar_wait(&xbar[xb], (xuse[xb]++) & 1u);
            uint8_t* xt = xin + xb * 2048 + lane * 64;
#pragma unroll
            for (int q = 0; q < 4; ++q) {
              float4* px = reinterpret_cast<float4*>(xt + ((q ^ sw) << 4));
              const float4 x4 = *px;
              float4 g4 = make_float4(1.f, 1.f, 1.f, 1.f);
              if (p.gate) g4 = *reinterpret_cast<const float4*>(wgate + k * 16 + 4 * q);
              const float4 y4 = make_float4(fmaf(__uint_as_float(r[k][4 * q + 0]), g4.x, x4.x), fmaf(__uint_as_float(r[k][4 * q + 1]), g4.y, x4.y),
                                            fmaf(__uint_as_float(r[k][4 * q + 2]), g4.z, x4.z), fmaf(__uint_as_float(r[k][4 * q + 3]), g4.w, x4.w));
              *px = y4;
              r[k][4 * q + 0] = __float_as_uint(y4.x); r[k][4 * q + 1] = __float_as_uint(y4.y);
              r[k][4 * q + 2] = __float_as_uint(y4.z); r[k][4 * q + 3] = __float_as_uint(y4.w);
            }
            fence_proxy_async();
            __syncwarp();
            if (lane == 0) {
              tma_store_2d(&tma_x, xin + xb * 2048, col, row0);
              tma_store_commit();
              if (k + 2 < NCH && ci + 2 * CP_CSETS < nchunks) {
                tma_store_wait_read<0>();
                mbar_expect_tx(&xbar[xb], 2048);
                tma_load_2d(xin + xb * 2048, &tma_x, &xbar[xb], col + 2 * CP_CSETS * 16, row0);
              }
            }
          }
          if (!fused_gn && !p.out_half) continue;
          if (lane == 0) tma_store_wait_read<0>();
          __syncwarp();
        }
        if (fused_gn) {
#pragma unroll
          for (int k = 0; k < NCH; ++k) {
            if (cset + CP_CSETS * k < nchunks) {
              float s0 = 0.f, q0 = 0.f;
#pragma unroll
              for (int j = 0; j < 16; ++j) {
                const float a = __uint_as_float(r[k][j]);
                s0 += a;
                q0 = fmaf(a, a, q0);
              }
#pragma unroll
              for (int off = 16; off > 0; off >>= 1) {
                s0 += __shfl_xor_sync(0xFFFFFFFFu, s0, off);
                q0 += __shfl_xor_sync(0xFFFFFFFFu, q0, off);
              }
              if (lane == 0) *reinterpret_cast<float2*>(stats + (quarter * 16 + cset + CP_CSETS * k) * 2) = make_float2(s0, q0);
            }
          }
          if (quarter < 2) asm volatile("bar.sync 2, %0;" ::"n"(CP_EPI_WARPS * 16) : "memory");
          else asm volatile("bar.sync 3, %0;" ::"n"(CP_EPI_WARPS * 16) : "memory");
        }
#pragma unroll
        for (int k = 0; k < NCH; ++k) {
          const int ci = cset + CP_CSETS * k;
          if (ci >= nchunks) break;
          const int col = cbase + ci * 16;
          if (fused_gn) {
            const float2 sa = *reinterpret_cast<const float2*>(stats + ((quarter & 2) * 16 + ci) * 2);
            const float2 sb = *reinterpret_cast<const float2*>(stats + ((quarter | 1) * 16 + ci) * 2);
            const float mean = (sa.x + sb.x) * (1.0f / 1024.0f);
            const float var = fmaxf((sa.y + sb.y) * (1.0f / 1024.0f) - mean * mean, 0.0f);
            const float rstd = rsqrtf(var + 1e-5f);
            float y[16];
#pragma unroll
            for (int q = 0; q < 4; ++q) {
              const float4 g4 = *reinterpret_cast<const float4*>(s_gamma + col + 4 * q);
              const float4 b4 = *reinterpret_cast<const float4*>(s_beta + col + 4 * q);
              y[4 * q + 0] = fmaf(__uint_as_float(r[k][4 * q + 0]) - mean, g4.x * rstd, b4.x);
              y[4 * q + 1] = fmaf(__uint_as_float(r[k][4 * q + 1]) - mean, g4.y * rstd, b4.y);
              y[4 * q + 2] = fmaf(__uint_as_float(r[k][4 * q + 2]) - mean, g4.z * rstd, b4.z);
              y[4 * q + 3] = fmaf(__uint_as_float(r[k][4 * q + 3]) - mean, g4.w * rstd, b4.w);
            }
            if (act == ACT_SILU) {
#pragma unroll
              for (int j = 0; j < 16; ++j) y[j] = __fdividef(y[j], 1.0f + __expf(-y[j]));
            } else if (act == ACT_RELU) {
#pragma unroll
              for (int j = 0; j < 16; ++j) y[j] = fmaxf(y[j], 0.0f);
            }
#pragma unroll
            for (int j = 0; j < 16; ++j) r[k][j] = __float_as_uint(y[j]);
          }
          if (p.out_tma && !want_prims) {
            if (p.pool_part && row0 < M) {
              float a8[8], a4[4], a2[2];
              const bool b4 = lane & 16, b3 = lane & 8, b2 = lane & 4, b1 = lane & 2;
#pragma unroll
              for (int j = 0; j < 8; ++j) {
                const float send = __uint_as_float(b4 ? r[k][j] : r[k][8 + j]), keep = __uint_as_float(b4 ? r[k][8 + j] : r[k][j]);
                a8[j] = keep + __shfl_xor_sync(0xFFFFFFFFu, send, 16);
              }
#pragma unroll
              for (int j = 0; j < 4; ++j) a4[j] = (b3 ? a8[4 + j] : a8[j]) + __shfl_xor_sync(0xFFFFFFFFu, b3 ? a8[j] : a8[4 + j], 8);
#pragma unroll
              for (int j = 0; j < 2; ++j) a2[j] = (b2 ? a4[2 + j] : a4[j]) + __shfl_xor_sync(0xFFFFFFFFu, b2 ? a4[j] : a4[2 + j], 4);
              float a1 = (b1 ? a2[1] : a2[0]) + __shfl_xor_sync(0xFFFFFFFFu, b1 ? a2[0] : a2[1], 2);
              a1 += __shfl_xor_sync(0xFFFFFFFFu, a1, 1);
              if (!(lane & 1)) p.pool_part[(size_t)(row0 >> 5) * p.N + col + (b4 ? 8 : 0) + (b3 ? 4 : 0) + (b2 ? 2 : 0) + (b1 ? 1 : 0)] = a1;
            }
            if (p.out_half) {
              uint8_t* tile = xout + (nstore & 1) * (FUSE == 2 ? 2048 : 1024);
              if (lane == 0) tma_store_wait_read<1>();
              __syncwarp();
              uint4 lo, hi;
              lo.x = pack_half2(__uint_as_float(r[k][0]), __uint_as_float(r[k][1]), p.fp16);
              lo.y = pack_half2(__uint_as_float(r[k][2]), __uint_as_float(r[k][3]), p.fp16);
              lo.z = pack_half2(__uint_as_float(r[k][4]), __uint_as_float(r[k][5]), p.fp16);
              lo.w = pack_half2(__uint_as_float(r[k][6]), __uint_as_float(r[k][7]), p.fp16);
              hi.x = pack_half2(__uint_as_float(r[k][8]), __uint_as_float(r[k][9]), p.fp16);
              hi.y = pack_half2(__uint_as_float(r[k][10]), __uint_as_float(r[k][11]), p.fp16);
              hi.z = pack_half2(__uint_as_float(r[k][12]), __uint_as_float(r[k][13]), p.fp16);
              hi.w = pack_half2(__uint_as_float(r[k][14]), __uint_as_float(r[k][15]), p.fp16);
              *reinterpret_cast<uint4*>(tile + lane * 32) = lo;
              *reinterpret_cast<uint4*>(tile + lane * 32 + 16) = hi;
              fence_proxy_async();
              __syncwarp();
              if (lane == 0) { tma_store_2d(&tma_out, tile, col, row0); tma_store_commit(); }
              ++nstore;
            } else {
              uint8_t* tile = xout;
              if (lane == 0) tma_store_wait_read<0>();
              __syncwarp();
#pragma unroll
              for (int q = 0; q < 4; ++q)
                *reinterpret_cast<uint4*>(tile + lane * 64 + q * 16) = make_uint4(r[k][4 * q], r[k][4 * q + 1], r[k][4 * q + 2], r[k][4 * q + 3]);
              fence_proxy_async();
              __syncwarp();
              if (lane == 0) { tma_store_2d(&tma_out, tile, col, row0); tma_store_commit(); }
            }
            continue;
          }
          const int sw = (lane >> 1) & 3;
#pragma unroll
          for (int q = 0; q < 4; ++q)
            *reinterpret_cast<uint4*>(stg + lane * 16 + ((q ^ sw) << 2)) = make_uint4(r[k][4 * q], r[k][4 * q + 1], r[k][4 * q + 2], r[k][4 * q + 3]);
          __syncwarp();
          if (p.pool_part && row0 < M) {
            const int c = lane & 15, par = lane >> 4;
            float cs_sum = 0.f;
#pragma unroll
            for (int i = 0; i < 16; ++i) {
              const int rr = 2 * i + par;
              cs_sum += stg[rr * 16 + ((((c >> 2) ^ ((rr >> 1) & 3)) << 2) | (c & 3))];
            }
            cs_sum += __shfl_xor_sync(0xFFFFFFFFu, cs_sum, 16);
            if (par == 0) p.pool_part[(size_t)(row0 >> 5) * p.N + col + c] = cs_sum;
          }
          if (want_prims && row0 < M) {
            const int c = lane & 15, par = lane >> 4, hb = quarter & 1;
            const int edge = hb ? 3 : 0;
            float tsum = 0.f, rsum = 0.f, c0 = 0.f, c7 = 0.f, k0 = 0.f, k7 = 0.f;
#pragma unroll
            for (int i = 0; i < 16; ++i) {
              const int rr = 2 * i + par;
              const float v = stg[rr * 16 + ((((c >> 2) ^ ((rr >> 1) & 3)) << 2) | (c & 3))];
              tsum += v;
              const bool on_edge = (i >> 2) == edge;
              rsum += on_edge ? v : 0.f;
              if ((i & 3) == 0) { c0 += par == 0 ? v : 0.f; k0 += (on_edge && par == 0) ? v : 0.f; }
              if ((i & 3) == 3) { c7 += par == 1 ? v : 0.f; k7 += (on_edge && par == 1) ? v : 0.f; }
            }
            tsum += __shfl_xor_sync(0xFFFFFFFFu, tsum, 16); rsum += __shfl_xor_sync(0xFFFFFFFFu, rsum, 16);
            c0 += __shfl_xor_sync(0xFFFFFFFFu, c0, 16); c7 += __shfl_xor_sync(0xFFFFFFFFu, c7, 16);
            k0 += __shfl_xor_sync(0xFFFFFFFFu, k0, 16); k7 += __shfl_xor_sync(0xFFFFFFFFu, k7, 16);
            __nv_bfloat16* pp = p.prims + (size_t)(row0 >> 5) * 6 * p.N + col + c;
            const float v0 = par ? c7 : tsum, v1 = par ? k0 : rsum, v2 = par ? k7 : c0;
            const int j0 = par ? 3 : 0, j1 = par ? 4 : 1, j2 = par ? 5 : 2;
            const uint32_t h01 = pack_half2(v0, v1, p.fp16), h2 = pack_half2(v2, 0.f, p.fp16);
            reinterpret_cast<uint16_t*>(pp)[(size_t)j0 * p.N] = (uint16_t)(h01 & 0xFFFFu);
            reinterpret_cast<uint16_t*>(pp)[(size_t)j1 * p.N] = (uint16_t)(h01 >> 16);
            reinterpret_cast<uint16_t*>(pp)[(size_t)j2 * p.N] = (uint16_t)(h2 & 0xFFFFu);
          }
          if (p.out_f32) {
            const int q = lane & 3;
#pragma unroll
            for (int i = 0; i < 4; ++i) {
              const int rr = (lane >> 2) + 8 * i;
              const int m = row0 + rr;
              if (m < M) {
                uint4 v = *reinterpret_cast<const uint4*>(stg + rr * 16 + ((q ^ ((rr >> 1) & 3)) << 2));
                *reinterpret_cast<uint4*>(p.out_f32 + (size_t)m * p.ldc + col + 4 * q) = v;
              }
            }
          }
          if (p.out_half) {
            const int hq = lane & 1;
#pragma unroll
            for (int i = 0; i < 2; ++i) {
              const int rr = (lane >> 1) + 16 * i;
              const int m = row0 + rr;
              if (m < M) {
                const int sw2 = (rr >> 1) & 3;
                float4 lo = *reinterpret_cast<const float4*>(stg + rr * 16 + (((2 * hq) ^ sw2) << 2));
                float4 hi = *reinterpret_cast<const float4*>(stg + rr * 16 + (((2 * hq + 1) ^ sw2) << 2));
                uint4 pk;
                pk.x = pack_half2(lo.x, lo.y, p.fp16); pk.y = pack_half2(lo.z, lo.w, p.fp16);
                pk.z = pack_half2(hi.x, hi.y, p.fp16); pk.w = pack_half2(hi.z, hi.w, p.fp16);
                *reinterpret_cast<uint4*>(p.out_half + (size_t)m * p.ldc + col + 8 * hq) = pk;
              }
            }
          }
          __syncwarp();
        }
      }
    }
    if (lane == 0) tma_store_wait_read<0>();
  }
  tc_fence_before();
  __syncthreads();
  cluster_sync_all();
  if (warp == 1) {
    tc_fence_after();
    tmem_dealloc_pair(tmem_base, 512);
  }
}

}
}
```

### matrix0_b200/csrc/tc_gemm.cuh

```cuda
#pragma once
#include <cuda.h>
#include <cuda_bf16.h>
#include <cuda_fp16.h>
#include "nn.cuh"

namespace m0 {
namespace tc {

static constexpr int BM = 128;
static constexpr int BK = 64;
static constexpr int A_TILE_BYTES = BM * BK * 2;
static constexpr int NUM_THREADS = 320;

__device__ __forceinline__ uint32_t smem_u32(const void* p) { return (uint32_t)__cvta_generic_to_shared(p); }

__device__ __forceinline__ void mbar_init(uint64_t* bar, uint32_t count) {
  asm volatile("mbarrier.init.shared::cta.b64 [%0], %1;" ::"r"(smem_u32(bar)), "r"(count) : "memory");
}
__device__ __forceinline__ void mbar_expect_tx(uint64_t* bar, uint32_t bytes) {
  asm volatile("mbarrier.arrive.expect_tx.shared::cta.b64 _, [%0], %1;" ::"r"(smem_u32(bar)), "r"(bytes) : "memory");
}
__device__ __forceinline__ void mbar_arrive(uint64_t* bar) {
  asm volatile("mbarrier.arrive.shared::cta.b64 _, [%0];" ::"r"(smem_u32(bar)) : "memory");
}
__device__ __forceinline__ void mbar_wait(uint64_t* bar, uint32_t parity) {
  asm volatile(
      "{\n\t"
      ".reg .pred p;\n\t"
      "WAIT_%=:\n\t"
      "mbarrier.try_wait.parity.shared::cta.b64 p, [%0], %1;\n\t"
      "@p bra DONE_%=;\n\t"
      "bra WAIT_%=;\n\t"
      "DONE_%=:\n\t"
      "}\n" ::"r"(smem_u32(bar)), "r"(parity)
      : "memory");
}
__device__ __forceinline__ void fence_barrier_init() { asm volatile("fence.mbarrier_init.release.cluster;" ::: "memory"); }
__device__ __forceinline__ void fence_proxy_async() { asm volatile("fence.proxy.async.shared::cta;" ::: "memory"); }

__device__ __forceinline__ void tma_prefetch_desc(const CUtensorMap* m) {
  asm volatile("prefetch.tensormap [%0];" ::"l"(reinterpret_cast<uint64_t>(m)) : "memory");
}
__device__ __forceinline__ void tma_load_2d(void* dst, const CUtensorMap* map, uint64_t* bar, int c0, int c1) {
  asm volatile("cp.async.bulk.tensor.2d.shared::cluster.global.mbarrier::complete_tx::bytes [%0], [%1, {%3, %4}], [%2];" ::"r"(smem_u32(dst)),
               "l"(reinterpret_cast<uint64_t>(map)), "r"(smem_u32(bar)), "r"(c0), "r"(c1)
               : "memory");
}
__device__ __forceinline__ void tma_load_4d(void* dst, const CUtensorMap* map, uint64_t* bar, int c0, int c1, int c2, int c3) {
  asm volatile("cp.async.bulk.tensor.4d.shared::cluster.global.mbarrier::complete_tx::bytes [%0], [%1, {%3, %4, %5, %6}], [%2];" ::"r"(
                   smem_u32(dst)),
               "l"(reinterpret_cast<uint64_t>(map)), "r"(smem_u32(bar)), "r"(c0), "r"(c1), "r"(c2), "r"(c3)
               : "memory");
}

__device__ __forceinline__ void tma_load_2d_mcast(void* dst, const CUtensorMap* map, uint64_t* bar, int c0, int c1, uint16_t cta_mask) {
  asm volatile(
      "cp.async.bulk.tensor.2d.shared::cluster.global.mbarrier::complete_tx::bytes.multicast::cluster [%0], [%1, {%3, %4}], [%2], %5;" ::"r"(
          smem_u32(dst)),
      "l"(reinterpret_cast<uint64_t>(map)), "r"(smem_u32(bar)), "r"(c0), "r"(c1), "h"(cta_mask)
      : "memory");
}
__device__ __forceinline__ bool elect_one() {
  uint32_t pred;
  asm volatile(
      "{\n\t"
      ".reg .pred P;\n\t"
      "elect.sync _|P, 0xFFFFFFFF;\n\t"
      "selp.u32 %0, 1, 0, P;\n\t"
      "}\n"
      : "=r"(pred));
  return pred != 0;
}
__device__ __forceinline__ uint32_t cluster_ctarank() {
  uint32_t r;
  asm volatile("mov.u32 %0, %%cluster_ctarank;" : "=r"(r));
  return r;
}
__device__ __forceinline__ void cluster_sync_all() {
  asm volatile("barrier.cluster.arrive.release.aligned;" ::: "memory");
  asm volatile("barrier.cluster.wait.acquire.aligned;" ::: "memory");
}

__device__ __forceinline__ void tmem_alloc(uint32_t* dst_smem, uint32_t cols) {
  asm volatile("tcgen05.alloc.cta_group::1.sync.aligned.shared::cta.b32 [%0], %1;" ::"r"(smem_u32(dst_smem)), "r"(cols) : "memory");
}
__device__ __forceinline__ void tmem_relinquish() { asm volatile("tcgen05.relinquish_alloc_permit.cta_group::1.sync.aligned;" ::: "memory"); }
__device__ __forceinline__ void tmem_dealloc(uint32_t addr, uint32_t cols) {
  asm volatile("tcgen05.dealloc.cta_group::1.sync.aligned.b32 %0, %1;" ::"r"(addr), "r"(cols) : "memory");
}
__device__ __forceinline__ void tc_fence_before() { asm volatile("tcgen05.fence::before_thread_sync;" ::: "memory"); }
__device__ __forceinline__ void tc_fence_after() { asm volatile("tcgen05.fence::after_thread_sync;" ::: "memory"); }

__device__ __forceinline__ void umma_bf16(uint32_t tmem_d, uint64_t desc_a, uint64_t desc_b, uint32_t idesc, uint32_t accumulate) {
  asm volatile(
      "{\n\t"
      ".reg .pred p;\n\t"
      "setp.ne.b32 p, %4, 0;\n\t"
      "tcgen05.mma.cta_group::1.kind::f16 [%0], %1, %2, %3, p;\n\t"
      "}\n" ::"r"(tmem_d),
      "l"(desc_a), "l"(desc_b), "r"(idesc), "r"(accumulate)
      : "memory");
}
__device__ __forceinline__ void umma_commit(uint64_t* bar) {
  asm volatile("tcgen05.commit.cta_group::1.mbarrier::arrive::one.shared::cluster.b64 [%0];" ::"r"(smem_u32(bar)) : "memory");
}
__device__ __forceinline__ void umma_commit_mcast(uint64_t* bar, uint16_t cta_mask) {
  asm volatile("tcgen05.commit.cta_group::1.mbarrier::arrive::one.shared::cluster.multicast::cluster.b64 [%0], %1;" ::"r"(smem_u32(bar)),
               "h"(cta_mask)
               : "memory");
}
__device__ __forceinline__ void tmem_ld_32x32(uint32_t taddr, uint32_t (&r)[32]) {
  asm volatile(
      "tcgen05.ld.sync.aligned.32x32b.x32.b32 "
      "{%0, %1, %2, %3, %4, %5, %6, %7, %8, %9, %10, %11, %12, %13, %14, %15, "
      "%16, %17, %18, %19, %20, %21, %22, %23, %24, %25, %26, %27, %28, %29, %30, %31}, [%32];"
      : "=r"(r[0]), "=r"(r[1]), "=r"(r[2]), "=r"(r[3]), "=r"(r[4]), "=r"(r[5]), "=r"(r[6]), "=r"(r[7]), "=r"(r[8]), "=r"(r[9]), "=r"(r[10]),
        "=r"(r[11]), "=r"(r[12]), "=r"(r[13]), "=r"(r[14]), "=r"(r[15]), "=r"(r[16]), "=r"(r[17]), "=r"(r[18]), "=r"(r[19]), "=r"(r[20]),
        "=r"(r[21]), "=r"(r[22]), "=r"(r[23]), "=r"(r[24]), "=r"(r[25]), "=r"(r[26]), "=r"(r[27]), "=r"(r[28]), "=r"(r[29]), "=r"(r[30]),
        "=r"(r[31])
      : "r"(taddr));
}
__device__ __forceinline__ void tmem_ld_wait() { asm volatile("tcgen05.wait::ld.sync.aligned;" ::: "memory"); }

__device__ __forceinline__ uint64_t make_smem_desc(uint32_t smem_addr) {
  return (uint64_t)((smem_addr >> 4) & 0x3FFFu) | (1ull << 16) | (64ull << 32) | (1ull << 46) | (2ull << 61);
}
__host__ __device__ __forceinline__ uint32_t make_idesc_bf16(int m, int n, int fp16 = 0) {
  const uint32_t fmt = fp16 ? 0u : 1u;
  return (1u << 4) | (fmt << 7) | (fmt << 10) | ((uint32_t)(n >> 3) << 17) | ((uint32_t)(m >> 4) << 24);
}

struct GemmParams {
  int M;
  int N;
  int n_store;
  int n_part;
  int taps;
  int kb_per_tap;
  int conv;
  int w_row0;
  int stages;
  int tmem_cols;
  int fp16;
  int cluster;
  float* out_f32;
  __nv_bfloat16* out_bf16;
  int ldc, col0;
  const float* bias;
  int act;
  float scale;
  const float* gn_gamma;
  const float* gn_beta;
  float* pool_part;
  int k_splits;
  long long split_stride;
  int n_slices;
  int acc_stages;
  int acc_stride;
};

__device__ __forceinline__ uint32_t pack_half2(float a, float b, int fp16) {
  if (fp16) {
    __half2 h = __floats2half2_rn(a, b);
    return *reinterpret_cast<uint32_t*>(&h);
  }
  __nv_bfloat162 t = __floats2bfloat162_rn(a, b);
  return *reinterpret_cast<uint32_t*>(&t);
}

__device__ __forceinline__ float tc_act(float x, int act) {
  switch (act) {
    case ACT_RELU: return x > 0.0f ? x : 0.0f;
    case ACT_SILU: return __fdividef(x, 1.0f + __expf(-x));
    case ACT_LEAKY: return x > 0.0f ? x : 0.05f * x;
    case ACT_TANH: return tanhf(x);
    case ACT_SIGMOID: return __fdividef(1.0f, 1.0f + __expf(-x));
    default: return x;
  }
}

static constexpr int EPI_STAGE_BYTES = 8 * 32 * 32 * 4 + 2 * 320 * 4 + 4 * 20 * 2 * 4;

__global__ void __launch_bounds__(NUM_THREADS, 1)
gemm_tc_kernel(const __grid_constant__ CUtensorMap tma_a, const __grid_constant__ CUtensorMap tma_w, const GemmParams p) {
  extern __shared__ __align__(1024) uint8_t smem_raw[];
  uint8_t* smem = reinterpret_cast<uint8_t*>((reinterpret_cast<uintptr_t>(smem_raw) + 1023) & ~uintptr_t(1023));
  const int w_tile_bytes = p.N * BK * 2;
  const int stage_bytes = A_TILE_BYTES + w_tile_bytes;
  float* epi_stage = reinterpret_cast<float*>(smem + (size_t)p.stages * stage_bytes);
  float* s_gamma = epi_stage + 8 * 32 * 32;
  float* s_beta = s_gamma + 320;
  float* s_stats = s_beta + 320;
  uint64_t* full_bar = reinterpret_cast<uint64_t*>(smem + (size_t)p.stages * stage_bytes + EPI_STAGE_BYTES);
  uint64_t* empty_bar = full_bar + p.stages;
  uint64_t* tmem_full_bar = empty_bar + p.stages;
  uint64_t* tmem_empty_bar = tmem_full_bar + 2;
  uint32_t* tmem_slot = reinterpret_cast<uint32_t*>(tmem_empty_bar + 2);
  const int na = p.acc_stages > 1 ? 2 : 1;

  const int warp = threadIdx.x >> 5, lane = threadIdx.x & 31;
  const int cs = p.cluster;
  const int rank = cs > 1 ? (int)cluster_ctarank() : 0;
  const int num_tiles = (p.M + BM - 1) / BM;
  const int num_groups = (num_tiles + cs - 1) / cs;
  const int num_clusters = gridDim.x / cs;
  const int cluster_id = blockIdx.x / cs;
  const int kblocks = p.taps * p.kb_per_tap;
  const int n_parts = p.N / p.n_part;
  const int slice_rows = p.n_part / cs;
  const int ns = p.n_slices > 1 ? p.n_slices : 1;
  const int nk = p.k_splits > 1 ? p.k_splits : 1;
  const int kb_part = kblocks / nk;
  const uint16_t mask = (uint16_t)((1u << cs) - 1u);

  if (warp == 0 && lane == 0) {
    tma_prefetch_desc(&tma_a);
    tma_prefetch_desc(&tma_w);
    for (int s = 0; s < p.stages; ++s) {
      mbar_init(&full_bar[s], 1);
      mbar_init(&empty_bar[s], (uint32_t)cs);
    }
    for (int a = 0; a < 2; ++a) {
      mbar_init(&tmem_full_bar[a], 1);
      mbar_init(&tmem_empty_bar[a], 256);
    }
    fence_barrier_init();
  }
  if (warp == 1) {
    tmem_alloc(tmem_slot, (uint32_t)p.tmem_cols);
    tmem_relinquish();
  }
  tc_fence_before();
  __syncthreads();
  if (cs > 1) cluster_sync_all();
  tc_fence_after();
  const uint32_t tmem_base = *tmem_slot;

  if (warp == 0) {
    if (lane == 0) {
      int stage = 0;
      uint32_t phase = 0;
      for (int gi = cluster_id; gi < num_groups * ns * nk; gi += num_clusters) {
        const int ks = gi % nk, gs = gi / nk;
        const int g = gs / ns, w_row0 = p.w_row0 + (gs - g * ns) * p.N;
        const int m0 = (g * cs + rank) * BM;
        for (int kb = ks * kb_part; kb < (ks + 1) * kb_part; ++kb) {
          mbar_wait(&empty_bar[stage], phase ^ 1);
          uint8_t* a_dst = smem + (size_t)stage * stage_bytes;
          uint8_t* w_dst = a_dst + A_TILE_BYTES;
          mbar_expect_tx(&full_bar[stage], (uint32_t)stage_bytes);
          const int tap = kb / p.kb_per_tap, kc = kb - tap * p.kb_per_tap;
          if (p.conv) {
            const int dy = tap / 3 - 1, dx = tap % 3 - 1;
            tma_load_4d(a_dst, &tma_a, &full_bar[stage], kc * BK, dx, dy, m0 >> 6);
          } else {
            tma_load_2d(a_dst, &tma_a, &full_bar[stage], kb * BK, m0);
          }
          for (int part = 0; part < n_parts; ++part) {
            uint8_t* dst = w_dst + ((size_t)part * p.n_part + (size_t)rank * slice_rows) * BK * 2;
            const int row = w_row0 + part * p.n_part + rank * slice_rows;
            if (cs > 1) tma_load_2d_mcast(dst, &tma_w, &full_bar[stage], kb * BK, row, mask);
            else tma_load_2d(dst, &tma_w, &full_bar[stage], kb * BK, row);
          }
          if (++stage == p.stages) { stage = 0; phase ^= 1; }
        }
      }
    }
  } else if (warp == 1) {
    const uint32_t idesc = make_idesc_bf16(BM, p.n_part, p.fp16);
    const uint32_t part_bytes = (uint32_t)(p.n_part * BK * 2);
    int stage = 0;
    uint32_t phase = 0, it = 0;
    const uint32_t smem_base = smem_u32(smem);
    for (int gi = cluster_id; gi < num_groups * ns * nk; gi += num_clusters, ++it) {
      const uint32_t acc = na == 2 ? (it & 1u) : 0u, acc_phase = na == 2 ? ((it >> 1) & 1u) : (it & 1u);
      const uint32_t tmem_acc = tmem_base + acc * (uint32_t)p.acc_stride;
      mbar_wait(&tmem_empty_bar[acc], acc_phase ^ 1);
      tc_fence_after();
      for (int kb = 0; kb < kb_part; ++kb) {
        mbar_wait(&full_bar[stage], phase);
        tc_fence_after();
        const uint32_t a_addr = smem_base + (uint32_t)stage * (uint32_t)stage_bytes;
        const uint64_t adesc0 = make_smem_desc(a_addr);
        const uint64_t bdesc0 = make_smem_desc(a_addr + A_TILE_BYTES);
        const uint64_t bdesc1 = make_smem_desc(a_addr + A_TILE_BYTES + part_bytes);
        if (elect_one()) {
          if (n_parts == 2) {
#pragma unroll
            for (int k = 0; k < BK / 16; ++k) {
              const uint32_t accum = (kb > 0 || k > 0) ? 1u : 0u;
              umma_bf16(tmem_acc, adesc0 + 2 * k, bdesc0 + 2 * k, idesc, accum);
              umma_bf16(tmem_acc + (uint32_t)p.n_part, adesc0 + 2 * k, bdesc1 + 2 * k, idesc, accum);
            }
          } else {
#pragma unroll
            for (int k = 0; k < BK / 16; ++k) umma_bf16(tmem_acc, adesc0 + 2 * k, bdesc0 + 2 * k, idesc, (kb > 0 || k > 0) ? 1u : 0u);
          }
          if (cs > 1) umma_commit_mcast(&empty_bar[stage], mask);
          else umma_commit(&empty_bar[stage]);
        }
        __syncwarp();
        if (++stage == p.stages) { stage = 0; phase ^= 1; }
      }
      if (elect_one()) umma_commit(&tmem_full_bar[acc]);
      __syncwarp();
    }
  } else {
    const int quarter = warp & 3;
    const int cset = (warp - 2) >> 2;
    float* stg = epi_stage + (warp - 2) * (32 * 32);
    const bool plain = (p.bias == nullptr) && (p.act == ACT_NONE) && (p.scale == 1.0f);
    const bool fused_gn = p.gn_gamma != nullptr;
    const int epi_tid = ((warp - 2) << 5) | lane;
    if (fused_gn) {
      for (int c = epi_tid; c < p.N; c += 256) { s_gamma[c] = p.gn_gamma[c]; s_beta[c] = p.gn_beta[c]; }
      asm volatile("bar.sync 1, 256;" ::: "memory");
    }
    uint32_t it = 0;
    for (int gi = cluster_id; gi < num_groups * ns * nk; gi += num_clusters, ++it) {
      const uint32_t acc = na == 2 ? (it & 1u) : 0u, acc_phase = na == 2 ? ((it >> 1) & 1u) : (it & 1u);
      const int ks = gi % nk, gs = gi / nk;
      const int g = gs / ns, slice = gs - g * ns;
      float* const out_f32 = p.out_f32 ? p.out_f32 + (size_t)ks * p.split_stride : nullptr;
      const int w_row0 = p.w_row0 + slice * p.N, col0 = p.col0 + slice * p.N;
      const int n_store = (p.n_store - slice * p.N) < p.N ? (p.n_store - slice * p.N) : p.N;
      mbar_wait(&tmem_full_bar[acc], acc_phase);
      tc_fence_after();
      const int tile_row0 = (g * cs + rank) * BM + quarter * 32;
      const uint32_t tmem_row = tmem_base + acc * (uint32_t)p.acc_stride + ((uint32_t)(quarter * 32) << 16);
      if (fused_gn) {
        for (int c0 = cset * 32; c0 < p.N; c0 += 64) {
          uint32_t r[32];
          tmem_ld_32x32(tmem_row + (uint32_t)c0, r);
          tmem_ld_wait();
          float s0 = 0.f, q0 = 0.f, s1 = 0.f, q1 = 0.f;
#pragma unroll
          for (int j = 0; j < 16; ++j) {
            float a = __uint_as_float(r[j]), b = __uint_as_float(r[16 + j]);
            s0 += a; q0 = fmaf(a, a, q0);
            s1 += b; q1 = fmaf(b, b, q1);
          }
#pragma unroll
          for (int off = 16; off > 0; off >>= 1) {
            s0 += __shfl_xor_sync(0xFFFFFFFFu, s0, off); q0 += __shfl_xor_sync(0xFFFFFFFFu, q0, off);
            s1 += __shfl_xor_sync(0xFFFFFFFFu, s1, off); q1 += __shfl_xor_sync(0xFFFFFFFFu, q1, off);
          }
          if (lane == 0) {
            float* st = s_stats + (quarter * 20 + (c0 >> 4)) * 2;
            st[0] = s0; st[1] = q0; st[2] = s1; st[3] = q1;
          }
        }
        if (quarter < 2) asm volatile("bar.sync 2, 128;" ::: "memory");
        else asm volatile("bar.sync 3, 128;" ::: "memory");
      }
      for (int c0 = cset * 32; c0 < p.N; c0 += 64) {
        uint32_t r[32];
        tmem_ld_32x32(tmem_row + (uint32_t)c0, r);
        tmem_ld_wait();
        if (fused_gn) {
          const int act = p.act;
#pragma unroll
          for (int h = 0; h < 2; ++h) {
            const int grp = (c0 >> 4) + h;
            const float* sa = s_stats + ((quarter & 2) * 20 + grp) * 2;
            const float* sb = s_stats + ((quarter | 1) * 20 + grp) * 2;
            const float mean = (sa[0] + sb[0]) * (1.0f / 1024.0f);
            const float var = fmaxf((sa[1] + sb[1]) * (1.0f / 1024.0f) - mean * mean, 0.0f);
            const float rstd = rsqrtf(var + 1e-5f);
#pragma unroll
            for (int j = 0; j < 16; ++j) {
              const int c = c0 + h * 16 + j;
              const float gm = s_gamma[c] * rstd;
              const float y = fmaf(__uint_as_float(r[h * 16 + j]) - mean, gm, s_beta[c]);
              r[h * 16 + j] = __float_as_uint(tc_act(y, act));
            }
          }
        } else if (!plain) {
          float bl = 0.0f;
          if (p.bias && c0 + lane < n_store) bl = __ldg(p.bias + w_row0 + c0 + lane);
          float x[32];
#pragma unroll
          for (int j = 0; j < 32; ++j) x[j] = __uint_as_float(r[j]) + __shfl_sync(0xFFFFFFFFu, bl, j);
          const int act = p.act;
          if (act == ACT_SIGMOID) {
#pragma unroll
            for (int j = 0; j < 32; ++j) x[j] = __fdividef(1.0f, 1.0f + __expf(-x[j]));
          } else if (act == ACT_SILU) {
#pragma unroll
            for (int j = 0; j < 32; ++j) x[j] = __fdividef(x[j], 1.0f + __expf(-x[j]));
          } else if (act == ACT_RELU) {
#pragma unroll
            for (int j = 0; j < 32; ++j) x[j] = fmaxf(x[j], 0.0f);
          } else if (act != ACT_NONE) {
#pragma unroll
            for (int j = 0; j < 32; ++j) x[j] = tc_act(x[j], act);
          }
          const float scale = p.scale;
#pragma unroll
          for (int j = 0; j < 32; ++j) r[j] = __float_as_uint(x[j] * scale);
        }
#pragma unroll
        for (int q = 0; q < 8; ++q)
          *reinterpret_cast<uint4*>(stg + lane * 32 + ((q ^ (lane & 7)) << 2)) = make_uint4(r[4 * q], r[4 * q + 1], r[4 * q + 2], r[4 * q + 3]);
        __syncwarp();
        const int ncols = (n_store - c0) < 32 ? (n_store - c0) : 32;
        if (p.pool_part && tile_row0 < p.M && lane < ncols) {
          float cs_sum = 0.f;
#pragma unroll
          for (int i = 0; i < 32; ++i) cs_sum += stg[i * 32 + ((((lane >> 2) ^ (i & 7)) << 2) | (lane & 3))];
          p.pool_part[(size_t)(tile_row0 >> 5) * p.N + c0 + lane] = cs_sum;
        }
        if (out_f32) {
          const int q = lane & 7;
#pragma unroll
          for (int i = 0; i < 8; ++i) {
            const int rr = (lane >> 3) + 4 * i;
            const int m = tile_row0 + rr;
            if (m < p.M && 4 * q < ncols) {
              uint4 v = *reinterpret_cast<const uint4*>(stg + rr * 32 + ((q ^ (rr & 7)) << 2));
              *reinterpret_cast<uint4*>(out_f32 + (size_t)m * p.ldc + col0 + c0 + 4 * q) = v;
            }
          }
        }
        if (p.out_bf16) {
          const int q2 = lane & 3;
#pragma unroll
          for (int i = 0; i < 4; ++i) {
            const int rr = (lane >> 2) + 8 * i;
            const int m = tile_row0 + rr;
            if (m < p.M && 8 * q2 < ncols) {
              float4 lo = *reinterpret_cast<const float4*>(stg + rr * 32 + (((2 * q2) ^ (rr & 7)) << 2));
              float4 hi = *reinterpret_cast<const float4*>(stg + rr * 32 + (((2 * q2 + 1) ^ (rr & 7)) << 2));
              uint4 pk;
              pk.x = pack_half2(lo.x, lo.y, p.fp16); pk.y = pack_half2(lo.z, lo.w, p.fp16);
              pk.z = pack_half2(hi.x, hi.y, p.fp16); pk.w = pack_half2(hi.z, hi.w, p.fp16);
              *reinterpret_cast<uint4*>(p.out_bf16 + (size_t)m * p.ldc + col0 + c0 + 8 * q2) = pk;
            }
          }
        }
        __syncwarp();
      }
      tc_fence_before();
      mbar_arrive(&tmem_empty_bar[acc]);
    }
  }
  tc_fence_before();
  __syncthreads();
  if (cs > 1) cluster_sync_all();
  if (warp == 1) {
    tc_fence_after();
    tmem_dealloc(tmem_base, (uint32_t)p.tmem_cols);
  }
}

}
}
```

Before: 14.02 million.

## Fuse squeeze-excitation FC1/FC2 gate into conv pair epilogue, drop split-K SE GEMMs

Computes the squeeze-excitation hidden layer and sigmoid gate directly inside the conv1+GroupNorm pair kernel epilogue. The per-board pooled primitives stay in shared memory instead of going to a global buffer, and the folded FC1 weights are applied there. This removes the separate split-K tensor-core GEMM, the tail/hidden kernels, their launches and the global round trip. The cost is extra CUDA-core FMA work and weight loads in the epilogue warps, plus a larger shared-memory epilogue that may reduce pipeline stages.

Measured after the change: 9.360 million (median of 6 runs). 0.668x the previous value.

```diff
diff --git a/matrix0_b200/csrc/nn_fused_kernels.cu b/matrix0_b200/csrc/nn_fused_kernels.cu
--- a/matrix0_b200/csrc/nn_fused_kernels.cu
+++ b/matrix0_b200/csrc/nn_fused_kernels.cu
@@ -309,68 +309,6 @@
   gn_act_res_kernel<<<B, C, 0, s>>>(x, gamma, beta, residual, residual_bstride, out, out_half, C, act, nn_half_format());
   return m0_check_launch("gn_act_res");
 }
-__global__ void se_hidden_kernel(const float* __restrict__ part, int splits, long long split_stride, const float* __restrict__ b1,
-                                 __nv_bfloat16* __restrict__ hidden, int B, int hid, int ld, int act, int fp16) {
-  const int i = blockIdx.x * blockDim.x + threadIdx.x;
-  if (i >= B * hid) return;
-  const int b = i / hid, u = i - b * hid;
-  float a = b1[u];
-  for (int ks = 0; ks < splits; ++ks) a += part[(size_t)ks * split_stride + (size_t)b * ld + u];
-  hidden[(size_t)b * ld + u] = fk_half(fk_act(a, act), fp16);
-}
-int nn_se_hidden(const float* part, int splits, long long split_stride, const float* b1, __nv_bfloat16* hidden, int B, int hid, int ld, int act,
-                 cudaStream_t s) {
-  se_hidden_kernel<<<(B * hid + 255) / 256, 256, 0, s>>>(part, splits, split_stride, b1, hidden, B, hid, ld, act, nn_half_format());
-  return m0_check_launch("se_hidden");
-}
-static constexpr int SE_TAIL_BOARDS = 8;
-__global__ void __launch_bounds__(320, 4)
-se_tail_kernel(const float* __restrict__ part, int splits, long long split_stride, int ld, const float* __restrict__ b1,
-                               const float* __restrict__ w2t, const float* __restrict__ b2, float* __restrict__ gate, int B, int C, int hid, int act) {
-  extern __shared__ __align__(16) float s_hid[];
-  const int b0 = blockIdx.x * SE_TAIL_BOARDS;
-  const int nb = min(SE_TAIL_BOARDS, B - b0);
-  for (int i = threadIdx.x; i < SE_TAIL_BOARDS * hid; i += blockDim.x) {
-    const int b = i / hid, u = i - b * hid;
-    float a = 0.f;
-    if (b < nb) {
-      a = b1[u];
-      for (int ks = 0; ks < splits; ++ks) a += part[(size_t)ks * split_stride + (size_t)(b0 + b) * ld + u];
-      a = fk_act(a, act);
-    }
-    s_hid[u * SE_TAIL_BOARDS + b] = a;
-  }
-  __syncthreads();
-  for (int c = threadIdx.x; c < C; c += blockDim.x) {
-    float acc[SE_TAIL_BOARDS];
-#pragma unroll
-    for (int b = 0; b < SE_TAIL_BOARDS; ++b) acc[b] = 0.f;
-    for (int u0 = 0; u0 < hid; u0 += 16) {
-      float w[16];
-#pragma unroll
-      for (int k = 0; k < 16; ++k) w[k] = (u0 + k < hid) ? __ldg(w2t + (size_t)(u0 + k) * C + c) : 0.f;
-#pragma unroll
-      for (int k = 0; k < 16; ++k) {
-        if (u0 + k >= hid) break;
-        const float4 h0 = *reinterpret_cast<const float4*>(s_hid + (u0 + k) * SE_TAIL_BOARDS);
-        const float4 h1 = *reinterpret_cast<const float4*>(s_hid + (u0 + k) * SE_TAIL_BOARDS + 4);
-        acc[0] = fmaf(w[k], h0.x, acc[0]); acc[1] = fmaf(w[k], h0.y, acc[1]); acc[2] = fmaf(w[k], h0.z, acc[2]); acc[3] = fmaf(w[k], h0.w, acc[3]);
-        acc[4] = fmaf(w[k], h1.x, acc[4]); acc[5] = fmaf(w[k], h1.y, acc[5]); acc[6] = fmaf(w[k], h1.z, acc[6]); acc[7] = fmaf(w[k], h1.w, acc[7]);
-      }
-    }
-    const float bias = b2[c];
-#pragma unroll
-    for (int b = 0; b < SE_TAIL_BOARDS; ++b)
-      if (b < nb) gate[(size_t)(b0 + b) * C + c] = __fdividef(1.0f, 1.0f + __expf(-(acc[b] + bias)));
-  }
-}
-int nn_se_tail(const float* part, int splits, long long split_stride, int ld, const float* b1, const float* w2t, const float* b2, float* gate, int B,
-               int C, int hid, int act, cudaStream_t s) {
-  const int threads = C >= 320 ? 320 : ((C + 31) / 32 * 32);
-  se_tail_kernel<<<(B + SE_TAIL_BOARDS - 1) / SE_TAIL_BOARDS, threads, (size_t)SE_TAIL_BOARDS * hid * sizeof(float), s>>>(
-      part, splits, split_stride, ld, b1, w2t, b2, gate, B, C, hid, act);
-  return m0_check_launch("se_tail");
-}
 __global__ void value_tail_kernel(const float* __restrict__ gate, const float* __restrict__ h, const float* __restrict__ w3, const float* __restrict__ b3,
                                   float* __restrict__ values, int B, int C) {
   const int b = blockIdx.x * (blockDim.x >> 5) + (threadIdx.x >> 5), lane = threadIdx.x & 31;
diff --git a/matrix0_b200/csrc/nn_tc_kernels.cu b/matrix0_b200/csrc/nn_tc_kernels.cu
--- a/matrix0_b200/csrc/nn_tc_kernels.cu
+++ b/matrix0_b200/csrc/nn_tc_kernels.cu
@@ -15,13 +15,9 @@
 int nn_se_apply_gn(const __nv_bfloat16* conv_out, const float* gate, float* x, const float* gamma, const float* beta, __nv_bfloat16* a_out, int B,
                    int C, int act, cudaStream_t s);
 int nn_planes_to_nhwc_half(const float* planes, __nv_bfloat16* out, int B, int P, cudaStream_t s);
-int nn_se_hidden(const float* part, int splits, long long split_stride, const float* b1, __nv_bfloat16* hidden, int B, int hid, int ld, int act,
-                 cudaStream_t s);
 int nn_gn_act_res(const float* x, const float* gamma, const float* beta, const float* residual, long long residual_bstride, float* out,
                   __nv_bfloat16* out_half, int B, int C, int act, cudaStream_t s);
 int nn_attention_tc(const void* qkv_half, const float* rel_bias, void* out_half, int B, int C, int heads, float mix, cudaStream_t s);
-int nn_se_tail(const float* part, int splits, long long split_stride, int ld, const float* b1, const float* w2t, const float* b2, float* gate, int B,
-               int C, int hid, int act, cudaStream_t s);
 int nn_value_tail(const float* gate, const float* h, const float* w3, const float* b3, float* values, int B, int C, cudaStream_t s);
 int nn_se_gate(const float* pool, const float* w1t, const float* b1, const float* w2t, const float* b2, float* gate, int B, int C, int hid, int act,
                cudaStream_t s);
@@ -149,7 +145,7 @@
 
 struct TcBlock {
   TcWeight conv1, conv2, qkv, proj;
-  TcWeight se_fold, se_w2;
+  __nv_bfloat16* se_fold = nullptr;
 };
 
 struct TcState {
@@ -162,12 +158,6 @@
   float *pool = nullptr, *se_hid = nullptr, *se_gate = nullptr;
   std::vector<float*> se_w1t, se_w2t;
   bool se_fused = false;
-  int hid_pad = 0;
-  __nv_bfloat16 *prims = nullptr, *se_hid_h = nullptr;
-  float* se_part = nullptr;
-  int se_splits = 1;
-  size_t se_rows = 0;
-  CUtensorMap prims_mat, se_hid_mat;
   __nv_bfloat16* planes_h = nullptr;
   __nv_bfloat16* qkv_h = nullptr;
   bool heads_tc = false;
@@ -283,7 +273,10 @@
 struct ConvFusion {
   float* resid_x = nullptr;
   const float* gate = nullptr;
-  __nv_bfloat16* prims = nullptr;
+  float* se_gate = nullptr;
+  const __nv_bfloat16* se_fold = nullptr;
+  const float *se_b1 = nullptr, *se_w2t = nullptr, *se_b2 = nullptr;
+  int se_hid = 0;
   const CUtensorMap* x_map = nullptr;
 };
 
@@ -306,13 +299,26 @@
   p.gn_gamma = gn_gamma;
   p.gn_beta = gn_beta;
   p.pool_part = pool_part;
-  if (fuse) { p.resid_x = fuse->resid_x; p.gate = fuse->gate; p.prims = fuse->prims; }
+  if (fuse) {
+    p.resid_x = fuse->resid_x;
+    p.gate = fuse->gate;
+    p.se_gate = fuse->se_gate;
+    p.se_fold = fuse->se_fold;
+    p.se_b1 = fuse->se_b1;
+    p.se_w2t = fuse->se_w2t;
+    p.se_b2 = fuse->se_b2;
+    p.se_hid = fuse->se_hid;
+    if (p.se_gate && (w.n_launch > tc::CP_SE_MAX_C || p.se_hid <= 0 || p.se_hid > tc::CP_SE_MAX_HID || !gn_gamma)) {
+      m0_set_error("pair kernel: the SE gate epilogue needs N <= %d, 0 < se_hidden <= %d and the GroupNorm epilogue", tc::CP_SE_MAX_C, tc::CP_SE_MAX_HID);
+      return M0_ERR_ARG;
+    }
+  }
   static int cap = -1;
   if (cap < 0) cap = env_int("M0_TC_STAGES", 0);
   const int stage_bytes = conv ? tc::CP_A_SLOT + 3 * (w.n_launch / 4) * 128 : (w.n_launch / 4) * 128;
   const int a_res = conv ? 0 : 2 * kblocks_for(cin) * tc::A_TILE_BYTES;
-  const int fz = !fuse ? 0 : fuse->resid_x ? 2 : fuse->prims ? 1 : 0;
-  const int epi_bytes = fz == 2 ? tc::CP_EPI_BYTES_FUSE : tc::CP_EPI_BYTES;
+  const int fz = !fuse ? 0 : fuse->resid_x ? 2 : fuse->se_gate ? 1 : 0;
+  const int epi_bytes = fz == 2 ? tc::CP_EPI_BYTES_FUSE : fz == 1 ? tc::CP_EPI_BYTES_SE : tc::CP_EPI_BYTES;
   int stages = (st->max_smem - 2048 - epi_bytes - a_res) / stage_bytes;
   if (stages > 8) stages = 8;
   if (cap > 0 && stages > cap) stages = cap;
@@ -346,7 +352,7 @@
   cfg.attrs = attr;
   cfg.numAttrs = 1;
   if (fuse && fuse->resid_x && (!fuse->x_map || (out_half && !out_map))) { m0_set_error("pair kernel: the residual epilogue needs the x and output tensor maps"); return M0_ERR_ARG; }
-  p.out_tma = (out_map && !(fuse && fuse->prims)) ? 1 : 0;
+  p.out_tma = (out_map && fz != 1) ? 1 : 0;
   M0_CUDA_TRY(cudaLaunchKernelEx(&cfg, kernel, a_map, w.map_pair, out_map ? *out_map : a_map, (fuse && fuse->x_map) ? *fuse->x_map : a_map, p));
   return m0_check_launch("conv_pair_kernel");
 }
@@ -387,19 +393,12 @@
 
 int launch_gemm(TcState* st, const CUtensorMap& a_map, const TcWeight& w, int M, int conv, int taps, int cin, int w_row0, int N, float* out_f32,
                 __nv_bfloat16* out_bf16, int ldc, int col0, const float* bias, int act, float scale, cudaStream_t s,
-                const float* gn_gamma = nullptr, const float* gn_beta = nullptr, float* pool_part = nullptr, int n_store = -1, int n_slices = 1,
-                int k_splits = 1, long long split_stride = 0) {
+                const float* gn_gamma = nullptr, const float* gn_beta = nullptr, float* pool_part = nullptr, int n_store = -1, int n_slices = 1) {
   tc::GemmParams p;
   memset(&p, 0, sizeof(p));
   p.M = M;
   p.N = N;
   p.n_slices = n_slices;
-  p.k_splits = k_splits;
-  p.split_stride = split_stride;
-  if (k_splits > 1 && (out_bf16 || bias || act != ACT_NONE || gn_gamma || pool_part || (taps * kblocks_for(cin)) % k_splits != 0 || !out_f32)) {
-    m0_set_error("tensor-core GEMM: split-K needs a plain fp32 output and a K range divisible into whole k-blocks");
-    return M0_ERR_ARG;
-  }
   p.n_store = n_store >= 0 ? n_store : N * n_slices;
   if (w.n_part > N || N % w.n_part != 0) { m0_set_error("tensor-core GEMM: launch width %d does not match the weight map box %d", N, w.n_part); return M0_ERR_ARG; }
   p.n_part = w.n_part;
@@ -447,7 +446,7 @@
   const int cs = w.cluster;
   const int groups = (tiles + cs - 1) / cs;
   int clusters = st->sm_count / cs;
-  if (clusters > groups * n_slices * k_splits) clusters = groups * n_slices * k_splits;
+  if (clusters > groups * n_slices) clusters = groups * n_slices;
   cudaLaunchConfig_t cfg;
   memset(&cfg, 0, sizeof(cfg));
   cfg.gridDim = dim3((unsigned)(clusters * cs));
@@ -501,11 +500,6 @@
   if (st->vf1_h) cudaFree(st->vf1_h);
   if (st->vf2_h) cudaFree(st->vf2_h);
   st->vf1_h = st->vf2_h = nullptr;
-  if (st->prims) cudaFree(st->prims);
-  if (st->se_hid_h) cudaFree(st->se_hid_h);
-  if (st->se_part) cudaFree(st->se_part);
-  st->se_part = nullptr;
-  st->prims = st->se_hid_h = nullptr;
   st->qkv_h = st->ph_h = st->pf_h = st->vh_h = nullptr;
   st->a1 = st->a2 = nullptr;
   st->pool = st->se_hid = st->se_gate = nullptr;
@@ -533,19 +527,6 @@
       TRY(make_map_2d(&st->vf2_mat, st->vf2_h, (uint64_t)need, C, 128));
     }
   }
-  if (st->se_fused && n->cfg.se) {
-    const size_t rows = ((size_t)need + 127) / 128 * 128;
-    M0_CUDA_TRY(cudaMalloc((void**)&st->prims, rows * 12 * C * 2));
-    M0_CUDA_TRY(cudaMalloc((void**)&st->se_hid_h, rows * st->hid_pad * 2));
-    M0_CUDA_TRY(cudaMemset(st->prims, 0, rows * 12 * C * 2));
-    M0_CUDA_TRY(cudaMemset(st->se_hid_h, 0, rows * st->hid_pad * 2));
-    const int kblocks = 12 * (int)C / 64;
-    st->se_splits = kblocks % 4 == 0 ? 4 : kblocks % 3 == 0 ? 3 : kblocks % 2 == 0 ? 2 : 1;
-    st->se_rows = rows;
-    M0_CUDA_TRY(cudaMalloc((void**)&st->se_part, (size_t)st->se_splits * rows * st->hid_pad * 4));
-    TRY(make_map_2d(&st->prims_mat, st->prims, rows, 12 * C, 128));
-    TRY(make_map_2d(&st->se_hid_mat, st->se_hid_h, rows, (uint64_t)st->hid_pad, 128));
-  }
   M0_CUDA_TRY(cudaMemset(st->planes_h, 0, (size_t)need * 64 * 64 * 2));
   TRY(make_map_nhwc(&st->planes_conv, st->planes_h, need, 64));
   TRY(make_map_nhwc(&st->planes_convp, st->planes_h, need, 64, 10));
@@ -637,26 +618,25 @@
       if (c.piece_square_tables && (rc = make_weight(st, &st->pst, n->w.pst_w, C, C, env_int("M0_TC_SLICE_PROJ", 1) ? slice_width_for(C, C) : C, s)) != M0_OK) break;
       if ((rc = make_weight(st, &st->inter, n->w.inter_w, C, 9 * C, C, s, 9)) != M0_OK) break;
     }
-    st->hid_pad = (c.se_hidden + 63) / 64 * 64;
-    st->se_fused = env_int("M0_TC_FUSE_SE", 1) != 0 && pair_ok(C) && (!c.se || c.se_hidden <= 256);
+    st->se_fused = env_int("M0_TC_FUSE_SE", 1) != 0 && pair_ok(C) && (!c.se || c.se_hidden <= tc::CP_SE_MAX_HID);
     st->blocks.resize(c.blocks);
     for (int i = 0; i < c.blocks && rc == M0_OK; ++i) {
       const m0_block_weights& b = n->w.blocks[i];
       if ((rc = make_weight(st, &st->blocks[i].conv1, b.conv1_w, C, 9 * C, C, s, 9)) != M0_OK) break;
       if ((rc = make_weight(st, &st->blocks[i].conv2, b.conv2_w, C, 9 * C, C, s, 9)) != M0_OK) break;
       if (st->se_fused && c.se) {
-        const int hid = c.se_hidden, hid16 = (hid + 15) / 16 * 16, K = 12 * C, hp = st->hid_pad;
-        float *fold = nullptr, *w2p = nullptr;
-        if ((rc = m0_check_cuda(cudaMalloc((void**)&fold, (size_t)hid16 * K * 4), "cudaMalloc se_fold")) != M0_OK) break;
-        st->allocs.push_back(fold);
-        if ((rc = m0_check_cuda(cudaMemsetAsync(fold, 0, (size_t)hid16 * K * 4, s), "memset se_fold")) != M0_OK) break;
-        if ((rc = m0_check_cuda(cudaMalloc((void**)&w2p, (size_t)C * hp * 4), "cudaMalloc se_w2")) != M0_OK) break;
-        st->allocs.push_back(w2p);
+        const int hid = c.se_hidden, K = 12 * C;
+        float* fold = nullptr;
+        void* fold_h = nullptr;
+        if ((rc = m0_check_cuda(cudaMalloc(&fold_h, (size_t)hid * K * 2), "cudaMalloc se_fold")) != M0_OK) break;
+        st->allocs.push_back(fold_h);
+        st->blocks[i].se_fold = (__nv_bfloat16*)fold_h;
+        if ((rc = m0_check_cuda(cudaMallocAsync((void**)&fold, (size_t)hid * K * 4, s), "cudaMallocAsync se_fold")) != M0_OK) break;
         se_fold_kernel<<<(hid * K + 255) / 256, 256, 0, s>>>(b.conv2_w, b.se_w1, fold, C, hid);
-        pad_cols_kernel<float><<<(C * hp + 255) / 256, 256, 0, s>>>(b.se_w2, w2p, C, hid, hp);
-        if ((rc = m0_check_launch("se_fold")) != M0_OK) break;
-        if ((rc = make_weight(st, &st->blocks[i].se_fold, fold, hid16, K, hid16, s)) != M0_OK) break;
-        if ((rc = make_weight(st, &st->blocks[i].se_w2, w2p, C, hp, C, s)) != M0_OK) break;
+        rc = m0_check_launch("se_fold");
+        if (rc == M0_OK) rc = nn_f32_to_bf16(fold, st->blocks[i].se_fold, (size_t)hid * K, s);
+        cudaFreeAsync(fold, s);
+        if (rc != M0_OK) break;
       }
       if (b.has_attention) {
         if ((rc = make_weight(st, &st->blocks[i].qkv, b.att_qkv_w, 3 * C, C, slice_width_for(3 * C, C), s)) != M0_OK) break;
@@ -692,9 +672,6 @@
     if (st->vh_h) cudaFree(st->vh_h);
     if (st->vf1_h) cudaFree(st->vf1_h);
     if (st->vf2_h) cudaFree(st->vf2_h);
-    if (st->prims) cudaFree(st->prims);
-    if (st->se_hid_h) cudaFree(st->se_hid_h);
-    if (st->se_part) cudaFree(st->se_part);
     delete st;
   }
   delete all;
@@ -755,29 +732,15 @@
     __nv_bfloat16* next_a = (fuse_next || run_att) ? st->a1 : nullptr;
     if (st->se_fused) {
       ConvFusion f1;
-      f1.prims = c.se ? st->prims : nullptr;
+      if (c.se) {
+        f1.se_gate = st->se_gate;
+        f1.se_fold = tb.se_fold;
+        f1.se_b1 = b.se_b1;
+        f1.se_w2t = st->se_w2t[i];
+        f1.se_b2 = b.se_b2;
+        f1.se_hid = c.se_hidden;
+      }
       PROF("conv1+gn", conv3x3(st, st->a1_conv, st->a1_convp, tb.conv1, B, C, nullptr, st->a2, act, s, b.gn2_w, b.gn2_b, nullptr, &f1));
-      if (c.se) {
-        static int se_nosplit = -1;
-        if (se_nosplit < 0) se_nosplit = env_int("M0_SE_NOSPLIT", 0);
-        if (se_nosplit) {
-          PROF("se_fc1", launch_gemm(st, st->prims_mat, tb.se_fold, B, 0, 1, 12 * C, 0, tb.se_fold.n, nullptr, st->se_hid_h, st->hid_pad, 0, b.se_b1, act, 1.0f, s,
-                                     nullptr, nullptr, nullptr, c.se_hidden));
-        } else {
-          PROF("se_fc1", launch_gemm(st, st->prims_mat, tb.se_fold, B, 0, 1, 12 * C, 0, tb.se_fold.n, st->se_part, nullptr, st->hid_pad, 0, none, ACT_NONE, 1.0f, s,
-                                     nullptr, nullptr, nullptr, c.se_hidden, 1, st->se_splits, (long long)st->se_rows * st->hid_pad));
-          static int se_tail = -1;
-          if (se_tail < 0) se_tail = env_int("M0_SE_TAIL", 1);
-          if (se_tail) {
-            PROF("se_tail", nn_se_tail(st->se_part, st->se_splits, (long long)st->se_rows * st->hid_pad, st->hid_pad, b.se_b1, st->se_w2t[i], b.se_b2,
-                                       st->se_gate, B, C, c.se_hidden, act, s));
-            goto se_done;
-          }
-          PROF("se_hidden", nn_se_hidden(st->se_part, st->se_splits, (long long)st->se_rows * st->hid_pad, b.se_b1, st->se_hid_h, B, c.se_hidden, st->hid_pad, act, s));
-        }
-        PROF("se_fc2", launch_gemm(st, st->se_hid_mat, tb.se_w2, B, 0, 1, st->hid_pad, 0, C, st->se_gate, nullptr, C, 0, b.se_b2, ACT_SIGMOID, 1.0f, s));
-      se_done:;
-      }
       ConvFusion f2;
       f2.resid_x = n->x;
       f2.gate = c.se ? st->se_gate : nullptr;
diff --git a/matrix0_b200/csrc/tc_conv_pair.cuh b/matrix0_b200/csrc/tc_conv_pair.cuh
--- a/matrix0_b200/csrc/tc_conv_pair.cuh
+++ b/matrix0_b200/csrc/tc_conv_pair.cuh
@@ -22,7 +22,12 @@
   float* pool_part;
   float* resid_x;
   const float* gate;
-  __nv_bfloat16* prims;
+  float* se_gate;
+  const __nv_bfloat16* se_fold;
+  const float* se_b1;
+  const float* se_w2t;
+  const float* se_b2;
+  int se_hid;
 };
 
 static constexpr int CP_EPI_WARP0 = 4;
@@ -33,6 +38,10 @@
 static constexpr int CP_A_SLOT = 160 * 128;
 static constexpr int CP_EPI_BYTES = CP_EPI_WARPS * 2048 + 2 * 512 * 4 + 2 * 4 * 16 * 2 * 4 + CP_EPI_WARPS * 64 * 4;
 static constexpr int CP_EPI_BYTES_FUSE = CP_EPI_BYTES + CP_EPI_WARPS * 2048;
+static constexpr int CP_SE_MAX_C = 320, CP_SE_MAX_HID = 256;
+static constexpr int CP_SE_UNITS = 5;
+static constexpr int CP_SE_W2_BATCH = 20;
+static constexpr int CP_EPI_BYTES_SE = CP_EPI_BYTES + 2 * 12 * CP_SE_MAX_C * 2 + 2 * CP_SE_MAX_HID * 4;
 
 __device__ __forceinline__ uint32_t mapa_u32(uint32_t addr, uint32_t rank) {
   uint32_t r;
@@ -88,6 +97,20 @@
   asm volatile("cp.async.bulk.tensor.2d.global.shared::cta.bulk_group [%0, {%2, %3}], [%1];" ::"l"(reinterpret_cast<uint64_t>(map)),
                "r"(smem_u32(smem_src)), "r"(c0), "r"(c1)
                : "memory");
+}
+__device__ __forceinline__ void unpack_half8(const uint4 v, int fp16, float (&f)[8]) {
+  const uint32_t w[4] = {v.x, v.y, v.z, v.w};
+#pragma unroll
+  for (int i = 0; i < 4; ++i) {
+    if (fp16) {
+      const float2 t = __half22float2(*reinterpret_cast<const __half2*>(&w[i]));
+      f[2 * i] = t.x;
+      f[2 * i + 1] = t.y;
+    } else {
+      f[2 * i] = __uint_as_float(w[i] << 16);
+      f[2 * i + 1] = __uint_as_float(w[i] & 0xFFFF0000u);
+    }
+  }
 }
 __device__ __forceinline__ void tma_store_commit() { asm volatile("cp.async.bulk.commit_group;" ::: "memory"); }
 template <int N>
@@ -114,7 +137,9 @@
   float* s_beta = s_gamma + 512;
   float* s_stats = s_beta + 512;
   float* s_gate = s_stats + 256;
-  uint64_t* full_bar = reinterpret_cast<uint64_t*>(s_gate + CP_EPI_WARPS * 64);
+  float* s_se_hid = s_gate + CP_EPI_WARPS * 64;
+  uint16_t* s_prims = reinterpret_cast<uint16_t*>(s_se_hid + (FUSE == 1 ? 2 * CP_SE_MAX_HID : 0));
+  uint64_t* full_bar = reinterpret_cast<uint64_t*>(s_prims + (FUSE == 1 ? 2 * 12 * CP_SE_MAX_C : 0));
   uint64_t* empty_bar = full_bar + p.stages;
   uint64_t* tmem_full_bar = empty_bar + p.stages;
   uint64_t* tmem_empty_bar = tmem_full_bar + 2;
@@ -268,7 +293,7 @@
     float* wgate = s_gate + (warp - CP_EPI_WARP0) * (NCH * 16);
     const bool fused_gn = p.gn_gamma != nullptr;
     const bool resid = FUSE == 2 && p.resid_x != nullptr;
-    const bool want_prims = FUSE == 1 && p.prims != nullptr;
+    const bool want_prims = FUSE == 1 && p.se_gate != nullptr;
     const int epi_tid = ((warp - CP_EPI_WARP0) << 5) | lane;
     const uint32_t lead_empty = mapa_u32(smem_u32(tmem_empty_bar), 0);
     const int nchunks = nh >> 4;
@@ -487,13 +512,13 @@
             tsum += __shfl_xor_sync(0xFFFFFFFFu, tsum, 16); rsum += __shfl_xor_sync(0xFFFFFFFFu, rsum, 16);
             c0 += __shfl_xor_sync(0xFFFFFFFFu, c0, 16); c7 += __shfl_xor_sync(0xFFFFFFFFu, c7, 16);
             k0 += __shfl_xor_sync(0xFFFFFFFFu, k0, 16); k7 += __shfl_xor_sync(0xFFFFFFFFu, k7, 16);
-            __nv_bfloat16* pp = p.prims + (size_t)(row0 >> 5) * 6 * p.N + col + c;
+            uint16_t* pp = s_prims + ((quarter >> 1) * 12 + hb * 6) * p.N + col + c;
             const float v0 = par ? c7 : tsum, v1 = par ? k0 : rsum, v2 = par ? k7 : c0;
             const int j0 = par ? 3 : 0, j1 = par ? 4 : 1, j2 = par ? 5 : 2;
             const uint32_t h01 = pack_half2(v0, v1, p.fp16), h2 = pack_half2(v2, 0.f, p.fp16);
-            reinterpret_cast<uint16_t*>(pp)[(size_t)j0 * p.N] = (uint16_t)(h01 & 0xFFFFu);
-            reinterpret_cast<uint16_t*>(pp)[(size_t)j1 * p.N] = (uint16_t)(h01 >> 16);
-            reinterpret_cast<uint16_t*>(pp)[(size_t)j2 * p.N] = (uint16_t)(h2 & 0xFFFFu);
+            pp[j0 * p.N] = (uint16_t)(h01 & 0xFFFFu);
+            pp[j1 * p.N] = (uint16_t)(h01 >> 16);
+            pp[j2 * p.N] = (uint16_t)(h2 & 0xFFFFu);
           }
           if (p.out_f32) {
             const int q = lane & 3;
@@ -526,6 +551,80 @@
           }
           __syncwarp();
         }
+        if (want_prims) {
+          asm volatile("bar.sync 4, %0;" ::"n"(CP_EPI_WARPS * 32) : "memory");
+          const int C8 = p.N >> 3, H8 = nh >> 3, hid = p.se_hid;
+          const uint4* P0 = reinterpret_cast<const uint4*>(s_prims);
+          const uint4* P1 = P0 + 12 * C8;
+          for (int u0 = warp - CP_EPI_WARP0; u0 < hid; u0 += CP_EPI_WARPS * CP_SE_UNITS) {
+            float a0[CP_SE_UNITS], a1[CP_SE_UNITS];
+#pragma unroll
+            for (int j = 0; j < CP_SE_UNITS; ++j) a0[j] = a1[j] = 0.f;
+#pragma unroll 1
+            for (int i = lane; i < 12 * H8; i += 32) {
+              const int sg = i / H8;
+              const int kk = sg * C8 + h * H8 + (i - sg * H8);
+              uint4 wv[CP_SE_UNITS];
+#pragma unroll
+              for (int j = 0; j < CP_SE_UNITS; ++j) {
+                const int u = u0 + j * CP_EPI_WARPS;
+                if (u < hid) wv[j] = __ldg(reinterpret_cast<const uint4*>(p.se_fold + (size_t)u * 12 * p.N) + kk);
+              }
+              const uint4 x0 = P0[kk], x1 = P1[kk];
+              float f0[8], f1[8];
+              unpack_half8(x0, p.fp16, f0);
+              unpack_half8(x1, p.fp16, f1);
+#pragma unroll
+              for (int j = 0; j < CP_SE_UNITS; ++j) {
+                if (u0 + j * CP_EPI_WARPS >= hid) break;
+                float w[8];
+                unpack_half8(wv[j], p.fp16, w);
+#pragma unroll
+                for (int e = 0; e < 8; ++e) { a0[j] = fmaf(w[e], f0[e], a0[j]); a1[j] = fmaf(w[e], f1[e], a1[j]); }
+              }
+            }
+#pragma unroll
+            for (int j = 0; j < CP_SE_UNITS; ++j) {
+#pragma unroll
+              for (int off = 16; off > 0; off >>= 1) {
+                a0[j] += __shfl_xor_sync(0xFFFFFFFFu, a0[j], off);
+                a1[j] += __shfl_xor_sync(0xFFFFFFFFu, a1[j], off);
+              }
+              const int u = u0 + j * CP_EPI_WARPS;
+              if (lane == 0 && u < hid) {
+                if (h == 0) {
+                  s_se_hid[u] = a0[j];
+                  s_se_hid[hid + u] = a1[j];
+                } else {
+                  const float b = __ldg(p.se_b1 + u);
+                  s_se_hid[u] = tc_act(b + (s_se_hid[u] + a0[j]), act);
+                  s_se_hid[hid + u] = tc_act(b + (s_se_hid[hid + u] + a1[j]), act);
+                }
+              }
+            }
+          }
+          if (h == 1) {
+            asm volatile("bar.sync 4, %0;" ::"n"(CP_EPI_WARPS * 32) : "memory");
+            const int gb = t * 4 + rank * 2;
+            for (int c = epi_tid; c < p.N; c += CP_EPI_WARPS * 32) {
+              float z0 = 0.f, z1 = 0.f;
+              for (int ub = 0; ub < hid; ub += CP_SE_W2_BATCH) {
+                float w[CP_SE_W2_BATCH];
+#pragma unroll
+                for (int j = 0; j < CP_SE_W2_BATCH; ++j) w[j] = ub + j < hid ? __ldg(p.se_w2t + (size_t)(ub + j) * p.N + c) : 0.f;
+#pragma unroll
+                for (int j = 0; j < CP_SE_W2_BATCH; ++j) {
+                  if (ub + j >= hid) break;
+                  z0 = fmaf(w[j], s_se_hid[ub + j], z0);
+                  z1 = fmaf(w[j], s_se_hid[hid + ub + j], z1);
+                }
+              }
+              const float bias = __ldg(p.se_b2 + c);
+              if (gb < p.boards) p.se_gate[(size_t)gb * p.N + c] = tc_act(z0 + bias, ACT_SIGMOID);
+              if (gb + 1 < p.boards) p.se_gate[(size_t)(gb + 1) * p.N + c] = tc_act(z1 + bias, ACT_SIGMOID);
+            }
+          }
+        }
       }
     }
     if (lane == 0) tma_store_wait_read<0>();
diff --git a/matrix0_b200/csrc/tc_gemm.cuh b/matrix0_b200/csrc/tc_gemm.cuh
--- a/matrix0_b200/csrc/tc_gemm.cuh
+++ b/matrix0_b200/csrc/tc_gemm.cuh
@@ -152,8 +152,6 @@
   const float* gn_gamma;
   const float* gn_beta;
   float* pool_part;
-  int k_splits;
-  long long split_stride;
   int n_slices;
   int acc_stages;
   int acc_stride;
@@ -209,8 +207,6 @@
   const int n_parts = p.N / p.n_part;
   const int slice_rows = p.n_part / cs;
   const int ns = p.n_slices > 1 ? p.n_slices : 1;
-  const int nk = p.k_splits > 1 ? p.k_splits : 1;
-  const int kb_part = kblocks / nk;
   const uint16_t mask = (uint16_t)((1u << cs) - 1u);
 
   if (warp == 0 && lane == 0) {
@@ -240,11 +236,10 @@
     if (lane == 0) {
       int stage = 0;
       uint32_t phase = 0;
-      for (int gi = cluster_id; gi < num_groups * ns * nk; gi += num_clusters) {
-        const int ks = gi % nk, gs = gi / nk;
-        const int g = gs / ns, w_row0 = p.w_row0 + (gs - g * ns) * p.N;
+      for (int gi = cluster_id; gi < num_groups * ns; gi += num_clusters) {
+        const int g = gi / ns, w_row0 = p.w_row0 + (gi - g * ns) * p.N;
         const int m0 = (g * cs + rank) * BM;
-        for (int kb = ks * kb_part; kb < (ks + 1) * kb_part; ++kb) {
+        for (int kb = 0; kb < kblocks; ++kb) {
           mbar_wait(&empty_bar[stage], phase ^ 1);
           uint8_t* a_dst = smem + (size_t)stage * stage_bytes;
           uint8_t* w_dst = a_dst + A_TILE_BYTES;
@@ -272,12 +267,12 @@
     int stage = 0;
     uint32_t phase = 0, it = 0;
     const uint32_t smem_base = smem_u32(smem);
-    for (int gi = cluster_id; gi < num_groups * ns * nk; gi += num_clusters, ++it) {
+    for (int gi = cluster_id; gi < num_groups * ns; gi += num_clusters, ++it) {
       const uint32_t acc = na == 2 ? (it & 1u) : 0u, acc_phase = na == 2 ? ((it >> 1) & 1u) : (it & 1u);
       const uint32_t tmem_acc = tmem_base + acc * (uint32_t)p.acc_stride;
       mbar_wait(&tmem_empty_bar[acc], acc_phase ^ 1);
       tc_fence_after();
-      for (int kb = 0; kb < kb_part; ++kb) {
+      for (int kb = 0; kb < kblocks; ++kb) {
         mbar_wait(&full_bar[stage], phase);
         tc_fence_after();
         const uint32_t a_addr = smem_base + (uint32_t)stage * (uint32_t)stage_bytes;
@@ -317,11 +312,10 @@
       asm volatile("bar.sync 1, 256;" ::: "memory");
     }
     uint32_t it = 0;
-    for (int gi = cluster_id; gi < num_groups * ns * nk; gi += num_clusters, ++it) {
+    for (int gi = cluster_id; gi < num_groups * ns; gi += num_clusters, ++it) {
       const uint32_t acc = na == 2 ? (it & 1u) : 0u, acc_phase = na == 2 ? ((it >> 1) & 1u) : (it & 1u);
-      const int ks = gi % nk, gs = gi / nk;
-      const int g = gs / ns, slice = gs - g * ns;
-      float* const out_f32 = p.out_f32 ? p.out_f32 + (size_t)ks * p.split_stride : nullptr;
+      const int g = gi / ns, slice = gi - g * ns;
+      float* const out_f32 = p.out_f32;
       const int w_row0 = p.w_row0 + slice * p.N, col0 = p.col0 + slice * p.N;
       const int n_store = (p.n_store - slice * p.N) < p.N ? (p.n_store - slice * p.N) : p.N;
       mbar_wait(&tmem_full_bar[acc], acc_phase);
```
